# antoyang/TubeDETR

Measured on AMD Instinct MI355X. Metric: training clips/sec (fwd+bwd) at T=100 k=4 res=352, 1/2/4/8 MI355X, higher is better.
Workload: dtype bf16

## Files before the change

### include/tubedetr_hip.h

```cpp
#ifndef TUBEDETR_HIP_H
#define TUBEDETR_HIP_H
#include <stddef.h>
#include <stdint.h>
#ifdef __cplusplus
extern "C" {
#endif

#define TD_F32 0
#define TD_BF16 1
#define TD_U8 2
#define TD_OK 0
#define TD_ERR_INVALID (-1)
#define TD_ERR_LAUNCH (-2)

typedef void* td_stream_t;

const char* td_last_error(void);
int td_abi_version(void);

int td_set_deterministic(int on);
int td_get_deterministic(void);


#define TD_PROF_GEMM_128x128 0
#define TD_PROF_GEMM_128x64 1
#define TD_PROF_WGRAD 2
#define TD_PROF_GEMM_64x128 3
#define TD_PROF_PW_RESIDENT 4
#define TD_PROF_GEMM_256 5
#define TD_PROF_GEMM_256_PW 6
#define TD_PROF_FUSED 7
#define TD_PROF_CROSS_Q1 8
#define TD_PROF_WGRAD_SINGLE 9
#define TD_PROF_CHAIN 10
#define TD_PROF_FAMILIES 11
int td_prof_enable(int on);
int td_prof_collect(int family, int dtype, long long* launches, double* ms, double* flops);
int td_prof_collect_bytes(int family, int dtype, double* bytes);
int td_prof_dump(const char* path);
int td_debug_set_stamp_buffer(unsigned long long* buf);

typedef struct td_conv_desc {
  int N, Hs, Ws, C;
  int Ho, Wo;
  int R, S, stride, pad;
  int mode;
  int Nc;
  int ldc;
  int out_sp;
  int out_H, out_W;
  int aniso;
  int stride_w, pad_w;
} td_conv_desc;

typedef struct td_epilogue {
  const float* bias;
  const void* residual;
  const void* mask_src;
  int relu;
  int sigmoid;
  float dropout_p;
  uint32_t dropout_seed;
  float alpha;
  const uint32_t* dropout_counter;
} td_epilogue;

int td_conv_gemm(const void* src, const void* wmat, void* out, const td_conv_desc* d, const td_epilogue* e,
                 int dtype, td_stream_t stream);

typedef struct td_linear_ex_desc {
  int M, N, K1, K2;
  int lda1, lda2, ldc, ldr;
  int w_shared;
  long long rows1, rows2;
  const int* a1_map;
  const int* a2_map;
  const int* out_map;
  const int* res_map;
} td_linear_ex_desc;
int td_linear_ex(const void* a1, const void* a2, const void* wmat, void* out, const td_linear_ex_desc* x, const td_epilogue* e,
                 int dtype, td_stream_t stream);

int td_conv_wgrad(const void* g, const void* src, float* dw, const td_conv_desc* d, int ldg, int dtype, int splits,
                  td_stream_t stream);
int td_conv_wgrad_bias(const void* g, const void* src, float* dw, float* dbias, const td_conv_desc* d, int ldg, int dtype,
                       int splits, td_stream_t stream);

typedef struct td_wgrad_job {
  const void* g;
  const void* src;
  float* dW;
  const float* scale;
  td_conv_desc d;
  int ldg;
  int ci_real;
  float* dbias;
  int accumulate;
  int prezeroed;
} td_wgrad_job;
size_t td_conv_wgrad_batch_table_bytes(int n_jobs);
int td_conv_wgrad_batch(const td_wgrad_job* jobs, int n_jobs, int dtype, void* table_host, void* table_dev, size_t table_bytes,
                        td_stream_t stream);

typedef struct td_frame_source {
  const void* data;
  int dtype;
  int n;
  const int* index;
  const int* valid_hw;
} td_frame_source;
int td_frames_to_nhwc(const td_frame_source* srcs, int n_srcs, int C, int H, int W, int Cpad, const float* mean,
                      const float* inv_std, void* y, int dtype, td_stream_t stream);

size_t td_resnet_fwd_ws_bytes(int N, int H, int W, const int* nblocks, int dtype, int save);
int td_resnet_num_convs(const int* nblocks);
int td_resnet_fwd(const td_frame_source* srcs, int n_srcs, const float* mean, const float* inv_std, int N, int H, int W,
                  const int* nblocks, const void* const* w_fwd, const float* const* bias, int save, void* ws, size_t ws_bytes,
                  void** feat, int* feat_hw, int stem_pairs, int first_train_stage, int dtype, td_stream_t stream);
int td_bottleneck_fused(const void* x, void* out, const void* w1, const float* b1, const void* w2, const float* b2, const void* w3,
                        const float* b3, const void* wd, const float* bd, int N, int H, int W, int Cin, int dtype, td_stream_t stream);
int td_pw_chain2(const void* y2, const void* w3, const float* b3, const void* residual, void* out, const void* w1, const float* b1,
                 void* h1, int M, int planes, int dtype, td_stream_t stream);
int td_stem_pair_weights(const void* w_fwd_8, void* w_pairs, int Co, int dtype, td_stream_t stream);
int td_stem_pool(const void* x_pairs, const void* w_pairs, const float* bias, void* pooled, int N, int H, int W, int dtype,
                 td_stream_t stream);
size_t td_resnet_bwd_ws_bytes(int N, int H, int W, const int* nblocks, int first_train_stage, int dtype);
size_t td_resnet_bwd_table_bytes(const int* nblocks, int first_train_stage);
int td_resnet_bwd(const void* dfeat, int N, int N_fwd, int H, int W, const int* nblocks, int first_train_stage,
                  const void* const* w_dgrad, const float* const* scale, float* const* dW, const void* fwd_ws, void* ws,
                  size_t ws_bytes, void* table_host, void* table_dev, size_t table_bytes, int dW_prezeroed, int dtype, int only_stage, td_stream_t stream);

int td_weight_prep(const float* W, const float* bn_w, const float* bn_b, const float* bn_rm, const float* bn_rv,
                   const float* bias, int Co, int Ci, int R, int S, int Cpad, void* w_fwd, void* w_dgrad,
                   float* bias_out, float* scale_out, int dtype, td_stream_t stream);

typedef struct td_prep_item {
  const float* W;
  const float *bn_w, *bn_b, *bn_rm, *bn_rv, *bias;
  void *w_fwd, *w_dgrad;
  float *bias_out, *scale_out;
  int Co, Ci, RS, Cpad, Co_alloc, blk0;
} td_prep_item;
int td_weight_prep_batch(const td_prep_item* items_dev, int n, int total_blocks, int dtype, td_stream_t stream);

int td_wgrad_finalize(const float* dw_k, const float* scale, float* dW, int Co, int Ci, int R, int S, int Cpad,
                      int accumulate, td_stream_t stream);

int td_nchw_to_nhwc(const float* x, void* y, int N, int C, int H, int W, int Cpad, int dtype, td_stream_t stream);
int td_nhwc_to_nchw(const void* x, float* y, int N, int C, int H, int W, int dtype, td_stream_t stream);
int td_cast(const void* x, void* y, size_t n, int src_dtype, int dst_dtype, td_stream_t stream);

// ... 106 lines not shown
```

### tubedetr_amd/_hip.py

```python
from __future__ import annotations

import ctypes as C
import os

import torch

TD_F32, TD_BF16 = 0, 1
EXPECTED_ABI = 11
_LIB_PATH = os.environ.get("TD_HIP_LIB") or os.path.join(os.path.dirname(os.path.abspath(__file__)), "lib", "libtubedetr_hip.so")
_lib = None


class ConvDesc(C.Structure):
    _fields_ = [(n, C.c_int) for n in ("N", "Hs", "Ws", "C", "Ho", "Wo", "R", "S", "stride", "pad", "mode", "Nc", "ldc", "out_sp", "out_H", "out_W",
                                       "aniso", "stride_w", "pad_w")]


class PrepItem(C.Structure):
    _fields_ = [(n, C.c_void_p) for n in ("W", "bn_w", "bn_b", "bn_rm", "bn_rv", "bias", "w_fwd", "w_dgrad", "bias_out", "scale_out")] + \
               [(n, C.c_int) for n in ("Co", "Ci", "RS", "Cpad", "Co_alloc", "blk0")]


class WgradJob(C.Structure):
    _fields_ = [("g", C.c_void_p), ("src", C.c_void_p), ("dW", C.c_void_p), ("scale", C.c_void_p), ("d", ConvDesc), ("ldg", C.c_int), ("ci_real", C.c_int), ("dbias", C.c_void_p), ("accumulate", C.c_int), ("prezeroed", C.c_int)]


TD_U8 = 2


class FrameSource(C.Structure):
    _fields_ = [("data", C.c_void_p), ("dtype", C.c_int), ("n", C.c_int), ("index", C.c_void_p), ("valid_hw", C.c_void_p)]


class LinearExDesc(C.Structure):
    _fields_ = [(n, C.c_int) for n in ("M", "N", "K1", "K2", "lda1", "lda2", "ldc", "ldr", "w_shared")] + \
               [("rows1", C.c_longlong), ("rows2", C.c_longlong)] + [(n, C.c_void_p) for n in ("a1_map", "a2_map", "out_map", "res_map")]


class OptimSegment(C.Structure):
    _fields_ = [("begin", C.c_longlong), ("end", C.c_longlong), ("group", C.c_int), ("active", C.c_int)]


class ResampleJob(C.Structure):
    _fields_ = [("src", C.c_void_p), ("src_frame_stride", C.c_longlong)] + [(n, C.c_int) for n in ("src_pitch", "T", "sh", "sw", "flip", "rh", "rw", "wy", "wx", "wh", "ww")] + \
               [("dst", C.c_void_p)] + [(n, C.c_int) for n in ("planar", "frame_off", "H", "W")] + [("mask", C.c_void_p)]


class Epilogue(C.Structure):
    _fields_ = [
        ("bias", C.c_void_p),
        ("residual", C.c_void_p),
        ("mask_src", C.c_void_p),
        ("relu", C.c_int),
        ("sigmoid", C.c_int),
        ("dropout_p", C.c_float),
        ("dropout_seed", C.c_uint32),
        ("alpha", C.c_float),
        ("dropout_counter", C.c_void_p),
    ]


_P, _I, _F, _U32, _SZ = C.c_void_p, C.c_int, C.c_float, C.c_uint32, C.c_size_t
_SIGS = {
    "td_prof_enable": [_I],
    "td_prof_dump": [C.c_char_p],
    "td_debug_set_stamp_buffer": [_P],
    "td_prof_collect": [_I, _I, C.POINTER(C.c_longlong), C.POINTER(C.c_double), C.POINTER(C.c_double)],
    "td_prof_collect_bytes": [_I, _I, C.POINTER(C.c_double)],
    "td_conv_gemm": [_P, _P, _P, C.POINTER(ConvDesc), C.POINTER(Epilogue), _I, _P],
    "td_conv_wgrad": [_P, _P, _P, C.POINTER(ConvDesc), _I, _I, _I, _P],
    "td_conv_wgrad_bias": [_P, _P, _P, _P, C.POINTER(ConvDesc), _I, _I, _I, _P],
    "td_conv_wgrad_batch": [C.POINTER(WgradJob), _I, _I, _P, _P, _SZ, _P],
    "td_resnet_num_convs": [C.POINTER(C.c_int)],
    "td_resnet_fwd": [C.POINTER(FrameSource), _I, C.POINTER(C.c_float), C.POINTER(C.c_float), _I, _I, _I, C.POINTER(C.c_int), C.POINTER(_P), C.POINTER(_P), _I, _P, _SZ,
                      C.POINTER(_P), C.POINTER(C.c_int), _I, _I, _I, _P],
    "td_bottleneck_fused": [_P, _P, _P, _P, _P, _P, _P, _P, _P, _P, _I, _I, _I, _I, _I, _P],
    "td_stem_pair_weights": [_P, _P, _I, _I, _P],
    "td_stem_pool": [_P, _P, _P, _P, _I, _I, _I, _I, _P],
    "td_pw_chain2": [_P, _P, _P, _P, _P, _P, _P, _P, _I, _I, _I, _P],
    "td_set_deterministic": [_I],
    "td_get_deterministic": [],
    "td_frames_to_nhwc": [C.POINTER(FrameSource), _I, _I, _I, _I, _I, C.POINTER(C.c_float), C.POINTER(C.c_float), _P, _I, _P],
    "td_resnet_bwd": [_P, _I, _I, _I, _I, C.POINTER(C.c_int), _I, C.POINTER(_P), C.POINTER(_P), C.POINTER(_P), _P, _P, _SZ, _P, _P, _SZ, _I, _I, _I, _P],
    "td_weight_prep_batch": [_P, _I, _I, _I, _P],
    "td_weight_prep": [_P, _P, _P, _P, _P, _P, _I, _I, _I, _I, _I, _P, _P, _P, _P, _I, _P],
    "td_wgrad_finalize": [_P, _P, _P, _I, _I, _I, _I, _I, _I, _P],
    "td_nchw_to_nhwc": [_P, _P, _I, _I, _I, _I, _I, _I, _P],
    "td_nhwc_to_nchw": [_P, _P, _I, _I, _I, _I, _I, _P],
    "td_cast": [_P, _P, _SZ, _I, _I, _P],
    "td_maxpool3x3s2": [_P, _P, _I, _I, _I, _I, _I, _P],
    "td_add_layernorm_fwd": [_P, _P, _P, _P, _P, _P, _P, _P, _I, _I, _F, _I, _P],
    "td_add_layernorm_bwd": [_P, _P, _P, _P, _P, _P, _P, _P, _P, _I, _I, _I, _P],
    "td_colsum": [_P, _P, _I, _I, _I, _I, _P],
    "td_add": [_P, _P, _P, _SZ, _I, _P],
    "td_relu_bwd": [_P, _P, _P, _SZ, _F, _I, _P],
    "td_gelu_fwd": [_P, _P, _SZ, _I, _P],
    "td_gelu_bwd": [_P, _P, _P, _SZ, _I, _P],
    "td_dropout": [_P, _P, _SZ, _F, _U32, _P, _I, _P],
    "td_pos_sine": [_P, _P, _I, _I, _I, _I, _F, _I, _I, _P],
    "td_linear_ex": [_P, _P, _P, _P, C.POINTER(LinearExDesc), C.POINTER(Epilogue), _I, _P],
    "td_rows_copy": [_P, _P, _P, _P, _P, _I, _I, _I, _I, _I, _I, _P],
    "td_rows_segment_sum": [_P, _P, _P, _P, _P, _I, _I, _I, _I, _I, _P],
    "td_criterion_fwd": [_P, _P, _P, _P, _P, _P, _P, _P, _P, _F, _F, _I, _I, _I, _I, _P, _P, _P, _P, _P, _P],
    "td_criterion_bwd": [_P, _P, _P, _P, _P, _P, _P, _P, _I, _I, _I, _P],
    "td_sted_decode": [_P, _P, _I, _I, _P],
    "td_grad_norm_clip": [_P, _SZ, C.POINTER(OptimSegment), _I, _F, _P, _SZ, _P, _P, _P],
    "td_adamw_ema_step": [_P, _P, _P, _P, _P, _SZ, C.POINTER(OptimSegment), _I, _P, _P, _P, _F, _F, _F, _F, _F, _P],
    "td_mha_fwd": [_P, _P, _P, _P, _P, _P, _P, _I, _I, _I, _I, _I, _I, _I, _I, _I, _F, _F, _U32, _P, _I, _P],
    "td_mha_bwd": [_P, _P, _P, _P, _P, _P, _P, _P, _P, _P, _I, _I, _I, _I, _I, _I, _I, _I, _I, _F, _F, _U32, _P, _I, _P],
    "td_cross_q1_fwd": [_P, _P, _P, _P, _P, _P, _P, _I, _I, _I, _I, _I, _F, _U32, _P, _I, _P],
    "td_cross_q1_bwd": [_P, _P, _P, _P, _P, _P, _P, _P, _I, _I, _I, _I, _I, _I, _F, _U32, _P, _I, _P],
    "td_cross_q1_bwd_coef": [_P, _P, _P, _P, _P, _P, _P, _P, _I, _I, _I, _I, _I, _I, _I, _F, _U32, _P, _I, _P],
    "td_cross_q1_dmem": [_P, _I, _P, _P, _I, _P, _I, _I, _I, _I, _I, _I, _P],
    "td_head_blocks_expand": [_P, _P, _F, _P, _P, _I, _I, _I, _P],
    "td_head_blocks_extract": [_P, _F, _P, _P, _I, _I, _P],
    "td_mha_lean_fwd": [_P, _P, _P, _P, _P, _P, _I, _I, _I, _I, _I, _I, _I, _I, _I, _F, _F, _U32, _P, _I, _P],
    "td_mha_lean_bwd": [_P, _P, _P, _P, _P, _P, _P, _P, _P, _P, _I, _I, _I, _I, _I, _I, _I, _I, _I, _F, _F, _U32, _P, _I, _P],
    "td_clip_resample": [C.POINTER(ResampleJob), _I, _P, _P, _SZ, _P],
}
_SIZE_SIGS = {
    "td_grad_norm_ws_bytes": [],
    "td_mha_lean_stats_bytes": [_I, _I, _I],
    "td_conv_wgrad_batch_table_bytes": [_I],
    "td_clip_resample_table_bytes": [_I],
    "td_resnet_bwd_table_bytes": [C.POINTER(C.c_int), _I],
    "td_resnet_fwd_ws_bytes": [_I, _I, _I, C.POINTER(C.c_int), _I, _I],
    "td_resnet_bwd_ws_bytes": [_I, _I, _I, C.POINTER(C.c_int), _I, _I],
}
EXPORTS = ["td_last_error", "td_abi_version"] + list(_SIGS) + list(_SIZE_SIGS)


def lib_path() -> str:
    return _LIB_PATH


def lib() -> C.CDLL:
    global _lib
    if _lib is None:
        if not os.path.exists(_LIB_PATH):
            raise RuntimeError(
                f"{_LIB_PATH} is missing: build it with `python -m tubedetr_amd.build` (or __graft_entry__.build()); "
                "tubedetr_amd has no CPU / eager fallback"
            )
        L = C.CDLL(_LIB_PATH)
        L.td_last_error.restype = C.c_char_p
        L.td_last_error.argtypes = []
        L.td_abi_version.restype = C.c_int
        L.td_abi_version.argtypes = []
        got = L.td_abi_version()
        if got != EXPECTED_ABI:
            raise RuntimeError(f"{_LIB_PATH} has ABI version {got}, this binding needs {EXPECTED_ABI}: rebuild it with "
                               "`python -m tubedetr_amd.build --force`")
# ... 35 lines not shown
```

### tubedetr_amd/csrc/gemm_conv.hip

```cpp
#include <stdlib.h>

#include <type_traits>

#include "td_common.h"
#include <algorithm>
#include <vector>

#ifndef TD_WGRAD_EARLY_ISSUE
#define TD_WGRAD_EARLY_ISSUE 1
#endif
#ifndef TD_BIG_XCD_CONTIG
#define TD_BIG_XCD_CONTIG 1
#endif
namespace td {

struct GemmParams {
  const char* src;
  const char* w;
  char* out;
  td_conv_desc d;
  int M, K;
  uint32_t src_bytes, w_bytes;
  unsigned long long* dbg;
  const float* bias;
  const char* residual;
  const char* mask_src;
  int relu, sigmoid;
  float alpha;
  uint32_t drop_thresh;
  float drop_scale;
  uint32_t seed;
  const uint32_t* seed_dev;
  const char* src2;
  uint32_t src2_bytes;
  int K1, lda1, lda2, ldr;
  int w_shared;
  const int* a1_map;
  const int* a2_map;
  const int* out_map;
  const int* res_map;
  int tap_inner;
  int w_ld;
  int wtap[4];
  int use_wtap;
};

template <typename T>
struct Mfma;
template <>
struct Mfma<u16> {
  static __device__ __forceinline__ void run(const uint4& wf, const uint4& af, f32x4& acc) {
    acc = __builtin_amdgcn_mfma_f32_16x16x32_bf16(*(const bf16x8*)&wf, *(const bf16x8*)&af, acc, 0, 0, 0);
  }
};
template <>
struct Mfma<float> {
  static __device__ __forceinline__ void run(const uint4& wf, const uint4& af, f32x4& acc) {
    const float* a = (const float*)&wf;
    const float* b = (const float*)&af;
#pragma unroll
    for (int s = 0; s < 4; ++s) acc = __builtin_amdgcn_mfma_f32_16x16x4f32(a[s], b[s], acc, 0, 0, 0);
  }
};

template <typename T>
__device__ __forceinline__ void load4(const char* base, size_t off, float (&o)[4]);
template <>
__device__ __forceinline__ void load4<float>(const char* base, size_t off, float (&o)[4]) {
  float4 v = *(const float4*)(base + off * 4);
  o[0] = v.x; o[1] = v.y; o[2] = v.z; o[3] = v.w;
}
template <>
__device__ __forceinline__ void load4<u16>(const char* base, size_t off, float (&o)[4]) {
  uint2 v = *(const uint2*)(base + off * 2);
  o[0] = __uint_as_float(v.x << 16); o[1] = __uint_as_float(v.x & 0xffff0000u);
  o[2] = __uint_as_float(v.y << 16); o[3] = __uint_as_float(v.y & 0xffff0000u);
}
template <typename T, typename V>
__device__ __forceinline__ void unpack4(const V& v, float (&o)[4]);
template <>
__device__ __forceinline__ void unpack4<float, float4>(const float4& v, float (&o)[4]) {
  o[0] = v.x; o[1] = v.y; o[2] = v.z; o[3] = v.w;
}
template <>
__device__ __forceinline__ void unpack4<u16, uint2>(const uint2& v, float (&o)[4]) {
  o[0] = __uint_as_float(v.x << 16); o[1] = __uint_as_float(v.x & 0xffff0000u);
  o[2] = __uint_as_float(v.y << 16); o[3] = __uint_as_float(v.y & 0xffff0000u);
}
typedef __bf16 bf16x2_t __attribute__((ext_vector_type(2)));
__device__ __forceinline__ uint32_t pack_bf16x2(float lo, float hi) {
  bf16x2_t v = {(__bf16)lo, (__bf16)hi};
  return *(uint32_t*)&v;
}
template <typename T>
__device__ __forceinline__ void unpack16(const uint4& v, float (&o)[16 / sizeof(T)]);
template <>
__device__ __forceinline__ void unpack16<float>(const uint4& v, float (&o)[4]) {
  o[0] = __uint_as_float(v.x); o[1] = __uint_as_float(v.y); o[2] = __uint_as_float(v.z); o[3] = __uint_as_float(v.w);
}
template <>
__device__ __forceinline__ void unpack16<u16>(const uint4& v, float (&o)[8]) {
  o[0] = __uint_as_float(v.x << 16); o[1] = __uint_as_float(v.x & 0xffff0000u);
  o[2] = __uint_as_float(v.y << 16); o[3] = __uint_as_float(v.y & 0xffff0000u);
  o[4] = __uint_as_float(v.z << 16); o[5] = __uint_as_float(v.z & 0xffff0000u);
  o[6] = __uint_as_float(v.w << 16); o[7] = __uint_as_float(v.w & 0xffff0000u);
}
template <typename T>
__device__ __forceinline__ uint4 pack16(const float (&v)[16 / sizeof(T)]);
template <>
__device__ __forceinline__ uint4 pack16<float>(const float (&v)[4]) {
  return make_uint4(__float_as_uint(v[0]), __float_as_uint(v[1]), __float_as_uint(v[2]), __float_as_uint(v[3]));
}
template <>
__device__ __forceinline__ uint4 pack16<u16>(const float (&v)[8]) {
  return make_uint4(pack_bf16x2(v[0], v[1]), pack_bf16x2(v[2], v[3]), pack_bf16x2(v[4], v[5]), pack_bf16x2(v[6], v[7]));
}
template <typename T>
__device__ __forceinline__ void store4(char* base, size_t off, const float (&v)[4]);
template <>
__device__ __forceinline__ void store4<float>(char* base, size_t off, const float (&v)[4]) {
  *(float4*)(base + off * 4) = make_float4(v[0], v[1], v[2], v[3]);
}
template <>
__device__ __forceinline__ void store4<u16>(char* base, size_t off, const float (&v)[4]) {
  uint2 o;
  o.x = (uint32_t)f32_to_bf16(v[0]) | ((uint32_t)f32_to_bf16(v[1]) << 16);
  o.y = (uint32_t)f32_to_bf16(v[2]) | ((uint32_t)f32_to_bf16(v[3]) << 16);
  *(uint2*)(base + off * 2) = o;
}

__device__ __forceinline__ float sigmoidf_(float x) { return 1.f / (1.f + __expf(-x)); }

typedef __attribute__((address_space(3))) void* lds_ptr_t;

#ifndef TD_NT
#define TD_NT 3
#endif
typedef uint32_t u32x4_t __attribute__((ext_vector_type(4)));
typedef uint32_t u32x2_t __attribute__((ext_vector_type(2)));
__device__ __forceinline__ uint4 ld16(const char* p) {
#if TD_NT & 1
  const u32x4_t v = __builtin_nontemporal_load((const u32x4_t*)p);
  return make_uint4(v.x, v.y, v.z, v.w);
#else
  return *(const uint4*)p;
#endif
}
__device__ __forceinline__ void st16(char* p, const uint4& v) {
#if TD_NT & 2
  __builtin_nontemporal_store(u32x4_t{v.x, v.y, v.z, v.w}, (u32x4_t*)p);
#else
  *(uint4*)p = v;
#endif
}

template <typename T, int BM, int BN, int NST, bool PW, bool TU = false, bool GX = false>
__global__ __launch_bounds__(256, (BM * BN >= 128 * 128 || NST == 3) ? 2 : 3) void conv_gemm_kernel(GemmParams p) {
  static_assert(!(PW && TU), "pointwise layers have no taps");
  static_assert(!GX || (PW && NST == 2), "the gather-extended operand is a pointwise, two-stage instance");
  constexpr int ES = sizeof(T);
  constexpr int VEC = 16 / ES;
  constexpr int BK = 128 / ES;
  constexpr int AI = BM / 32, BI = BN / 32;
  constexpr int WM = BM / 2, WN = BN / 2;
  constexpr int TM = WM / 16, TN = WN / 16;
  constexpr uint32_t OOB = 0xFFFFFFF0u;
  __shared__ __attribute__((aligned(16))) char smem0[(BM + BN) * 128];
  __shared__ __attribute__((aligned(16))) char smem1[(BM + BN) * 128];
  __shared__ __attribute__((aligned(16))) char smem2[NST == 3 ? (BM + BN) * 128 : 16];

  const td_conv_desc& d = p.d;
  const int t = threadIdx.x;
  const int wave = __builtin_amdgcn_readfirstlane(t >> 6), lane = t & 63;
  const int NT = (d.Nc + BN - 1) / BN;
  const int xcd = blockIdx.x & 7, seq = blockIdx.x >> 3;
  const int mt = (seq / NT) * 8 + xcd, nt = seq - (seq / NT) * NT;
  const int m0 = mt * BM, n0 = nt * BN;
  if (m0 >= p.M) return;
  const int lrow = lane >> 3;
  const int chunk = (lane & 7) ^ lrow;
  const int HoWo = d.Ho * d.Wo;

  const __amdgpu_buffer_rsrc_t rs_src = __builtin_amdgcn_make_buffer_rsrc((void*)p.src, 0, p.src_bytes, 0x00020000);
  const __amdgpu_buffer_rsrc_t rs_w = __builtin_amdgcn_make_buffer_rsrc((void*)p.w, 0, p.w_bytes, 0x00020000);
  const __amdgpu_buffer_rsrc_t rs_src2 = __builtin_amdgcn_make_buffer_rsrc((void*)(GX ? p.src2 : p.src), 0, GX ? p.src2_bytes : p.src_bytes, 0x00020000);

  int a_img[AI], a_hb[AI], a_wb[AI];
  bool a_ok[AI];
  uint32_t a_off[AI];
  uint32_t a_off2[GX ? AI : 1];
  int a_base[AI];
  uint32_t a_mask[AI];
  const int RS = d.R * d.S;
#pragma unroll
  for (int i = 0; i < AI; ++i) {
    int m = m0 + (i * 4 + wave) * 8 + lrow;
    a_ok[i] = m < p.M;
    if constexpr (GX) {
      const int mm = a_ok[i] ? m : 0;
      const int r1 = p.a1_map ? p.a1_map[mm] : mm;
      const int r2 = p.a2_map ? p.a2_map[mm] : mm;
      a_off[i] = a_ok[i] ? (uint32_t)r1 * (uint32_t)p.lda1 * ES : OOB;
      a_off2[i] = (a_ok[i] && p.src2) ? (uint32_t)r2 * (uint32_t)p.lda2 * ES : OOB;
    } else if constexpr (PW) {
      a_off[i] = a_ok[i] ? (uint32_t)m * (uint32_t)p.K * ES : OOB;
    } else {
      int mm = a_ok[i] ? m : 0;
      int n = mm / HoWo;
      int rem = mm - n * HoWo;
      int ho = rem / d.Wo, wo = rem - ho * d.Wo;
      a_img[i] = n * d.Hs * d.Ws;
      if (d.mode == 0) {
        a_hb[i] = ho * d.stride - d.pad;
        a_wb[i] = d.aniso ? wo * d.stride_w - d.pad_w : wo * d.stride - d.pad;
      } else {
        a_hb[i] = ho + d.pad;
        a_wb[i] = wo + d.pad;
      }
      if constexpr (TU) {
        a_base[i] = a_img[i] + a_hb[i] * d.Ws + a_wb[i];
        uint32_t msk = 0;
        for (int r = 0; r < d.R; ++r) {
          const int hs = d.mode == 0 ? a_hb[i] + r : a_hb[i] - r;
          for (int sx = 0; sx < d.S; ++sx) {
            const int ws = d.mode == 0 ? a_wb[i] + sx : a_wb[i] - sx;
            const bool in = (unsigned)hs < (unsigned)d.Hs && (unsigned)ws < (unsigned)d.Ws;
            msk |= (in ? 1u : 0u) << (r * d.S + sx);
          }
        }
        a_mask[i] = a_ok[i] ? msk : 0u;
      }
    }
  }
  uint32_t b_off[BI];
#pragma unroll
  for (int i = 0; i < BI; ++i) {
    int n = n0 + (i * 4 + wave) * 8 + lrow;
    b_off[i] = n < d.Nc ? (uint32_t)n * (uint32_t)(p.w_ld ? p.w_ld : ((GX && p.w_shared) ? p.K1 : p.K)) * ES : OOB;
  }
// ... 163 lines not shown
    for (int kt = 0; kt < nk; kt += 2) {
      __syncthreads();
      if (kt == 0) TD_STAMP(1);
      if (kt + 1 < nk) issue_tile(smem1);
      compute_tile(smem0);
      if (kt + 1 >= nk) break;
      __syncthreads();
      if (kt + 2 < nk) issue_tile(smem0);
      compute_tile(smem1);
    }
    TD_STAMP(2);
    fetch_epilogue_operands();
  } else {
#define TD_CG_STEP(cur, nxt, j)                                                     \
  asm volatile("s_waitcnt vmcnt(%0)" ::"n"(AI + BI) : "memory");                    \
  __builtin_amdgcn_s_barrier();                                                     \
  issue_tile(nxt);                                                                  \
  if ((j) >= 0) compute_tile(cur);
    for (int it = -2; it < nk; it += 3) {
      TD_CG_STEP(smem1, smem0, it)
      if (it + 1 >= nk) break;
      TD_CG_STEP(smem2, smem1, it + 1)
      if (it + 2 >= nk) break;
      TD_CG_STEP(smem0, smem2, it + 2)
    }
#undef TD_CG_STEP
    asm volatile("s_waitcnt vmcnt(0)" ::: "memory");
    TD_STAMP(2);
    fetch_epilogue_operands();
  }

  asm volatile("s_waitcnt lgkmcnt(0)" ::: "memory");
  __builtin_amdgcn_s_barrier();
  TD_STAMP(3);
  float* stg = (float*)((wave < 2 ? smem0 : smem1) + (wave & 1) * (WM * WN * 4));
  const float alpha = p.alpha;
#pragma unroll
  for (int j = 0; j < TM; ++j) {
    const int row = j * 16 + lr;
#pragma unroll
    for (int i = 0; i < TN; ++i) {
      const int c = (i * 4 + lg) ^ (row & (CPRW - 1));
      f32x4 a = acc[i][j];
      *(float4*)(stg + row * WN + c * 4) = make_float4(a[0] * alpha, a[1] * alpha, a[2] * alpha, a[3] * alpha);
    }
  }
  asm volatile("s_waitcnt lgkmcnt(0)" ::: "memory");
  float bias[EPL];
#pragma unroll
  for (int r = 0; r < EPL; ++r) bias[r] = (p.bias && n + r < d.Nc) ? p.bias[n + r] : 0.f;
  TD_STAMP(4);
  const uint32_t eff_seed = effective_seed(p.seed, p.drop_thresh ? p.seed_dev : nullptr);
#pragma unroll
  for (int it = 0; it < NIT; ++it) {
    if (!live[it]) continue;
    const int row = it * RPI + rsub;
    const int sw = row & (CPRW - 1);
    float v[EPL];
#pragma unroll
    for (int q = 0; q < EPL / 4; ++q) {
      float4 f = *(const float4*)(stg + row * WN + (((cc * (EPL / 4) + q) ^ sw) * 4));
      v[4 * q + 0] = f.x + bias[4 * q + 0]; v[4 * q + 1] = f.y + bias[4 * q + 1];
      v[4 * q + 2] = f.z + bias[4 * q + 2]; v[4 * q + 3] = f.w + bias[4 * q + 3];
    }
    const size_t off = offs[it];
    if (vec_ok) {
      if (p.residual) {
        float r8[EPL];
        unpack16<T>(res[it], r8);
#pragma unroll
        for (int r = 0; r < EPL; ++r) v[r] += r8[r];
      }
      if (p.relu) {
#pragma unroll
        for (int r = 0; r < EPL; ++r) v[r] = fmaxf(v[r], 0.f);
      }
      if (p.sigmoid) {
#pragma unroll
        for (int r = 0; r < EPL; ++r) v[r] = sigmoidf_(v[r]);
      }
      if (p.mask_src) {
        float m8[EPL];
        unpack16<T>(msk[it], m8);
#pragma unroll
        for (int r = 0; r < EPL; ++r) v[r] = m8[r] > 0.f ? v[r] : 0.f;
      }
      if (p.drop_thresh) {
#pragma unroll
        for (int r = 0; r < EPL; ++r) v[r] = dropout_keep(eff_seed, (uint32_t)(off + r), p.drop_thresh) ? v[r] * p.drop_scale : 0.f;
      }
      st16(p.out + off * ES, pack16<T>(v));
    } else {
      const int cnt = min(EPL, d.Nc - n);
      for (int r = 0; r < cnt; ++r) {
        float x = v[r];
        if (p.residual) x += Elem<T>::load(p.residual, (GX ? roffs[it] : off) + r);
        if (p.relu) x = fmaxf(x, 0.f);
        if (p.sigmoid) x = sigmoidf_(x);
        if (p.mask_src) x = Elem<T>::load(p.mask_src, off + r) > 0.f ? x : 0.f;
        if (p.drop_thresh) x = dropout_keep(eff_seed, (uint32_t)(off + r), p.drop_thresh) ? x * p.drop_scale : 0.f;
        Elem<T>::store(p.out, off + r, x);
      }
    }
  }
  TD_STAMP(5);
#undef TD_STAMP
}

#ifndef TD_ABL
#define TD_ABL 0
#endif
template <int OFF>
__device__ __forceinline__ u32x4_t lds_read16(uint32_t addr) {
  u32x4_t r;
#if TD_ABL & 4
  asm volatile("" : "=v"(r) : "v"(addr));
#else
  asm volatile("ds_read_b128 %0, %1 offset:%2" : "=v"(r) : "v"(addr), "n"(OFF));
#endif
  return r;
}
template <int N>
__device__ __forceinline__ void wait_vmcnt() {
  asm volatile("s_waitcnt vmcnt(%0)" ::"n"(N) : "memory");
}
template <int I>
using ic = std::integral_constant<int, I>;

#ifndef TD_BIG8_AUX_W
#define TD_BIG8_AUX_W 0
#endif
#ifndef TD_BIG8_AUX_X
#define TD_BIG8_AUX_X 0
#endif
template <bool TU, bool RES>
__global__ __launch_bounds__(512, 1) void conv_gemm_big8_kernel(GemmParams p) {
  using T = u16;
  constexpr int ES = 2, BM = 256, BN = 256, BK = 64, NW = 8, VEC = 8;
  constexpr int WM = 128, WN = 64, TM = 8, TN = 4;
  constexpr int STAGE = (BM + BN) * 128, WREG = BM * 128;
  constexpr uint32_t OOB = 0xFFFFFFF0u;
  constexpr int MAXT = 160;
  constexpr int STG = 16 * WN * ES;
  __shared__ __attribute__((aligned(16))) char smem[2 * STAGE];
  __shared__ __attribute__((aligned(16))) uint4 ktab[MAXT];
  __shared__ __attribute__((aligned(16))) char stg_all[NW * STG];

  const td_conv_desc& d = p.d;
  const int t = threadIdx.x;
  const int wave = __builtin_amdgcn_readfirstlane(t >> 6), lane = t & 63;
  const int NT = d.Nc / BN;
  const int lrow = lane >> 3;
  const int chunk = (lane & 7) ^ lrow;
  const int HoWo = d.Ho * d.Wo;
  const __amdgpu_buffer_rsrc_t rs_src = __builtin_amdgcn_make_buffer_rsrc((void*)p.src, 0, p.src_bytes, 0x00020000);
  const __amdgpu_buffer_rsrc_t rs_w = __builtin_amdgcn_make_buffer_rsrc((void*)p.w, 0, p.w_bytes, 0x00020000);
  const uint32_t out_bytes = (uint32_t)p.M * (uint32_t)d.ldc * ES;
  const __amdgpu_buffer_rsrc_t rs_out = __builtin_amdgcn_make_buffer_rsrc((void*)p.out, 0, out_bytes, 0x00020000);
  const int wy = wave >> 2, wx = wave & 3;
  const int RS = d.R * d.S;
  const int lane_c = chunk * VEC;
  const int nk = p.K / BK;
  const bool tap_inner = TU && p.tap_inner;
  if (t < nk + 4) {
    uint32_t xo, tap = 0, wo;
    if constexpr (TU) {
      const int cpt = d.C / BK;
      const int chunkc = tap_inner ? t / RS : t % cpt;
// ... 185 lines not shown
#pragma unroll
    for (int i = 0; i < TN; ++i) bs[i] = p.bias ? *(const f32x4*)(p.bias + n0 + wx * WN + i * 16 + lg * 4) : f32x4{0.f, 0.f, 0.f, 0.f};
    wait_vmcnt<7>();
    __builtin_amdgcn_s_barrier();
    if (wy == 1) __builtin_amdgcn_s_barrier();
    TD_STAMP(1);
    const int npair = (nk + 1) / 2;
#pragma unroll 1
    for (int it = 0; it < npair; ++it) {
      phase(ic<0>{}, ic<0>{}); phase(ic<0>{}, ic<1>{}); phase(ic<0>{}, ic<2>{}); phase(ic<0>{}, ic<3>{});
      phase(ic<1>{}, ic<0>{}); phase(ic<1>{}, ic<1>{}); phase(ic<1>{}, ic<2>{}); phase(ic<1>{}, ic<3>{});
    }
    if (wy == 0) __builtin_amdgcn_s_barrier();
    TD_STAMP(2);
    asm volatile("s_waitcnt vmcnt(0) lgkmcnt(0)" ::: "memory");
    asm volatile("s_nop 15\n\ts_nop 15" ::: "memory");
#pragma unroll
    for (int i = 0; i < TN; ++i)
#pragma unroll
      for (int j = 0; j < TM; ++j) asm volatile("" : "+v"(acc[i][j]));
#pragma unroll
    for (int i = 0; i < TN; ++i) asm volatile("" : "+v"(bs[i]));
    const int vb_next = vb + (int)gridDim.x;
    const bool more = tile_ok(vb_next);
    if (more) {
      tile_addr(tile_m0(vb_next), tile_n0(vb_next));
      prologue_issue();
    }
    TD_STAMP(3);
    uint4 mk[2][2];
    auto seg_off = [&](int j, int h) -> uint32_t {
      const int m = m0 + wy * WM + j * 16 + h * 8 + rsub;
      return m < p.M ? ((uint32_t)m * (uint32_t)d.ldc + (uint32_t)(n0 + wx * WN + cc * 8)) * ES : OOB;
    };
    auto fetch_mask = [&](int j, int b) {
#pragma unroll
      for (int h = 0; h < 2; ++h) {
        const uint32_t off = seg_off(j, h);
        mk[b][h] = off != OOB ? ld16(p.mask_src + off) : make_uint4(0, 0, 0, 0);
      }
    };
    auto put = [&](int j) {
#pragma unroll
      for (int i = 0; i < TN; ++i) {
        const f32x4 a = acc[i][j];
        float v[4] = {a[0] * alpha + bs[i][0], a[1] * alpha + bs[i][1], a[2] * alpha + bs[i][2], a[3] * alpha + bs[i][3]};
        if constexpr (RES) {
          const int m = m0 + wy * WM + j * 16 + lr;
          if (m < p.M) {
            const uint2 rr = *(const uint2*)(p.residual + ((size_t)m * d.ldc + n0 + wx * WN + i * 16 + lg * 4) * ES);
            v[0] += __uint_as_float(rr.x << 16); v[1] += __uint_as_float(rr.x & 0xffff0000u);
            v[2] += __uint_as_float(rr.y << 16); v[3] += __uint_as_float(rr.y & 0xffff0000u);
          }
        }
        if (p.relu) {
#pragma unroll
          for (int r = 0; r < 4; ++r) v[r] = fmaxf(v[r], 0.f);
        }
        const uint32_t lo = pack_bf16x2(v[0], v[1]), hi = pack_bf16x2(v[2], v[3]);
        asm volatile("ds_write_b64 %0, %1" ::"v"(swa[i]), "v"(u32x2_t{lo, hi}) : "memory");
      }
    };
    if (p.mask_src) fetch_mask(0, 0);
    put(0);
    u32x4_t o0, o1;
    asm volatile("ds_read_b128 %0, %1" : "=v"(o0) : "v"(sra) : "memory");
    asm volatile("ds_read_b128 %0, %1 offset:1024" : "=v"(o1) : "v"(sra) : "memory");
#pragma unroll
    for (int j = 0; j < TM; ++j) {
      const int b = j & 1;
      if (j + 1 < TM) {
        if (p.mask_src) fetch_mask(j + 1, b ^ 1);
        put(j + 1);
        asm volatile("s_waitcnt lgkmcnt(4)" : "+v"(o0), "+v"(o1) : : "memory");
      } else {
        asm volatile("s_waitcnt lgkmcnt(0)" : "+v"(o0), "+v"(o1) : : "memory");
      }
      u32x4_t s0 = o0, s1 = o1;
      if (j + 1 < TM) {
        asm volatile("ds_read_b128 %0, %1" : "=v"(o0) : "v"(sra) : "memory");
        asm volatile("ds_read_b128 %0, %1 offset:1024" : "=v"(o1) : "v"(sra) : "memory");
      }
      if (p.mask_src) {
        float x8[8], m8[8];
        unpack16<T>(make_uint4(s0.x, s0.y, s0.z, s0.w), x8);
        unpack16<T>(mk[b][0], m8);
#pragma unroll
        for (int r = 0; r < 8; ++r) x8[r] = m8[r] > 0.f ? x8[r] : 0.f;
        const uint4 q0 = pack16<T>(x8);
        s0 = u32x4_t{q0.x, q0.y, q0.z, q0.w};
        unpack16<T>(make_uint4(s1.x, s1.y, s1.z, s1.w), x8);
        unpack16<T>(mk[b][1], m8);
#pragma unroll
        for (int r = 0; r < 8; ++r) x8[r] = m8[r] > 0.f ? x8[r] : 0.f;
        const uint4 q1 = pack16<T>(x8);
        s1 = u32x4_t{q1.x, q1.y, q1.z, q1.w};
      }
      __builtin_amdgcn_raw_buffer_store_b128(s0, rs_out, (int)seg_off(j, 0), 0, 0);
      __builtin_amdgcn_raw_buffer_store_b128(s1, rs_out, (int)seg_off(j, 1), 0, 0);
    }
    TD_STAMP(5);
    if (p.dbg && t == 0) p.dbg[(size_t)vb * 8 + 7] = wall_clock64();
    if (!more) break;
    vb = vb_next;
  }
#undef TD_STAMP
}

template <bool TU>
__global__ __launch_bounds__(512, 1) void conv_gemm_big8n_kernel(GemmParams p) {
  using T = u16;
  constexpr int ES = 2, BM = 256, BN = 128, BK = 64, NW = 8, VEC = 8;
  constexpr int WM = 64, WN = 64, TM = 4, TN = 4;
  constexpr int WREG = BM * 128, STAGE = (BM + BN) * 128;
  constexpr uint32_t OOB = 0xFFFFFFF0u;
  constexpr int MAXT = 160;
  __shared__ __attribute__((aligned(16))) char smem[3 * STAGE];
  __shared__ __attribute__((aligned(16))) uint4 ktab[MAXT];

  const td_conv_desc& d = p.d;
  const int t = threadIdx.x;
  const int wave = __builtin_amdgcn_readfirstlane(t >> 6), lane = t & 63;
  const int NT = d.Nc / BN;
  const int xcd = blockIdx.x & 7, seq = blockIdx.x >> 3;
#if TD_BIG_XCD_CONTIG
  const int mtx = (cdiv(p.M, BM) + 7) / 8;
  const int mt = xcd * mtx + seq / NT, nt = seq - (seq / NT) * NT;
#else
  const int mt = (seq / NT) * 8 + xcd, nt = seq - (seq / NT) * NT;
#endif
  const int m0 = mt * BM, n0 = nt * BN;
  if (m0 >= p.M) return;
  const int lrow = lane >> 3;
  const int chunk = (lane & 7) ^ lrow;
  const int lane_c = chunk * VEC;
  const int HoWo = d.Ho * d.Wo;
  const int RS = d.R * d.S;
  const __amdgpu_buffer_rsrc_t rs_src = __builtin_amdgcn_make_buffer_rsrc((void*)p.src, 0, p.src_bytes, 0x00020000);
  const __amdgpu_buffer_rsrc_t rs_w = __builtin_amdgcn_make_buffer_rsrc((void*)p.w, 0, p.w_bytes, 0x00020000);
  const int wy = wave >> 1, wx = wave & 1;
  const int grp = wave >> 2;

  uint32_t a_off[4], a_mask[4];
  const float rcp_howo = 1.f / (float)HoWo, rcp_wo = 1.f / (float)d.Wo;
  auto divmod = [](int a, int dv, float rcp, int& q, int& r) {
    q = (int)((float)a * rcp);
    r = a - q * dv;
    const int up = r >= dv, dn = r < 0;
    q += up - dn;
    r += (dn - up) * dv;
  };
#pragma unroll
  for (int q = 0; q < 4; ++q) {
    const int m = m0 + (wave >> 1) * WM + (q >> 1) * 32 + ((wave & 1) * 2 + (q & 1)) * 8 + lrow;
    const bool ok = m < p.M;
    if constexpr (!TU) {
      a_off[q] = ((uint32_t)m * (uint32_t)p.K + (uint32_t)lane_c) * ES;
      a_mask[q] = ok ? 1u : 0u;
    } else {
      const int mm = ok ? m : 0;
      int n, rem, ho, wo;
      divmod(mm, HoWo, rcp_howo, n, rem);
      divmod(rem, d.Wo, rcp_wo, ho, wo);
      const int hb = d.mode == 0 ? ho * d.stride - d.pad : ho + d.pad;
      const int wb = d.mode == 0 ? wo * d.stride - d.pad : wo + d.pad;
      a_off[q] = ((uint32_t)(n * d.Hs * d.Ws + hb * d.Ws + wb) * (uint32_t)d.C + (uint32_t)lane_c) * ES;
      uint32_t cols = 0, msk = 0;
      for (int sx = 0; sx < d.S; ++sx) cols |= ((unsigned)(d.mode == 0 ? wb + sx : wb - sx) < (unsigned)d.Ws ? 1u : 0u) << sx;
      for (int r = 0; r < d.R; ++r) msk |= ((unsigned)(d.mode == 0 ? hb + r : hb - r) < (unsigned)d.Hs ? cols : 0u) << (r * d.S);
      a_mask[q] = ok ? msk : 0u;
    }
  }
  uint32_t b_off[2];
#pragma unroll
  for (int i = 0; i < 2; ++i) b_off[i] = ((uint32_t)(n0 + (i * NW + wave) * 8 + lrow) * (uint32_t)p.K + (uint32_t)lane_c) * ES;
  const int nk = p.K / BK;
  const bool tap_inner = TU && p.tap_inner;
// ... 97 lines not shown
      if (p.residual) res[b][it] = ld16(p.residual + offs[b][it] * ES);
      if (p.mask_src) msk[b][it] = ld16(p.mask_src + offs[b][it] * ES);
    }
  };

#define TD_STAMP(i) do { if (p.dbg && t == 0) p.dbg[(size_t)blockIdx.x * 8 + (i)] = __builtin_readcyclecounter(); } while (0)
  TD_STAMP(0);
  __syncthreads();
  {
    const u32x4_t e0 = lds_read16<0>(tab0);
    const u32x4_t e1 = lds_read16<16>(tab0);
    e[2] = lds_read16<32>(tab0);
    asm volatile("s_waitcnt lgkmcnt(0)" ::: "memory");
    __builtin_amdgcn_sched_barrier(0);
    issue_w(smem, 0, e0); issue_w(smem, 1, e0); issue_x(smem, 0, e0); issue_x(smem, 1, e0); issue_x(smem, 2, e0); issue_x(smem, 3, e0);
    issue_w(smem + STAGE, 0, e1); issue_w(smem + STAGE, 1, e1); issue_x(smem + STAGE, 0, e1); issue_x(smem + STAGE, 1, e1);
    issue_x(smem + STAGE, 2, e1); issue_x(smem + STAGE, 3, e1);
  }
  wait_vmcnt<8>();
  __builtin_amdgcn_s_barrier();
  if (grp == 1) __builtin_amdgcn_s_barrier();
  TD_STAMP(1);
  const int ntri = (nk + 2) / 3;
#pragma unroll 1
  for (int it = 0; it < ntri; ++it) {
    phase(ic<0>{}, ic<0>{}); phase(ic<0>{}, ic<1>{});
    phase(ic<1>{}, ic<0>{}); phase(ic<1>{}, ic<1>{});
    phase(ic<2>{}, ic<0>{}); phase(ic<2>{}, ic<1>{});
  }
  if (grp == 0) __builtin_amdgcn_s_barrier();
  TD_STAMP(2);
  asm volatile("s_waitcnt vmcnt(0) lgkmcnt(0)" ::: "memory");
  asm volatile("s_nop 15\n\ts_nop 15" ::: "memory");
#pragma unroll
  for (int i = 0; i < TN; ++i)
#pragma unroll
    for (int j = 0; j < TM; ++j) asm volatile("" : "+v"(acc[i][j]));
  fetch_chunk(0, 0);
  __builtin_amdgcn_s_barrier();
  TD_STAMP(3);
  float* stg = (float*)(smem + wave * (CR * WN * 4));
  const float alpha = p.alpha;
  float bias[EPL];
#pragma unroll
  for (int r = 0; r < EPL; ++r) bias[r] = p.bias ? p.bias[n + r] : 0.f;
#pragma unroll
  for (int c = 0; c < NCH; ++c) {
    const int b = c & 1;
    {
      const int row = lr;
#pragma unroll
      for (int i = 0; i < TN; ++i) {
        const int cx = (i * 4 + lg) ^ (row & (CPRW - 1));
        const f32x4 a = acc[i][c];
        *(float4*)(stg + row * WN + cx * 4) = make_float4(a[0] * alpha, a[1] * alpha, a[2] * alpha, a[3] * alpha);
      }
    }
    if (c + 1 < NCH) fetch_chunk(c + 1, b ^ 1);
    asm volatile("s_waitcnt lgkmcnt(0)" ::: "memory");
#pragma unroll
    for (int it = 0; it < NIT; ++it) {
      const int row = it * RPI + rsub;
      const int sw = row & (CPRW - 1);
      float v[EPL];
#pragma unroll
      for (int q = 0; q < EPL / 4; ++q) {
        const float4 f = *(const float4*)(stg + row * WN + (((cc * (EPL / 4) + q) ^ sw) * 4));
        v[4 * q + 0] = f.x + bias[4 * q + 0]; v[4 * q + 1] = f.y + bias[4 * q + 1];
        v[4 * q + 2] = f.z + bias[4 * q + 2]; v[4 * q + 3] = f.w + bias[4 * q + 3];
      }
      if (p.residual) {
        float r8[EPL];
        unpack16<T>(res[b][it], r8);
#pragma unroll
        for (int r = 0; r < EPL; ++r) v[r] += r8[r];
      }
      if (p.relu) {
#pragma unroll
        for (int r = 0; r < EPL; ++r) v[r] = fmaxf(v[r], 0.f);
      }
      if (p.mask_src) {
        float m8[EPL];
        unpack16<T>(msk[b][it], m8);
#pragma unroll
        for (int r = 0; r < EPL; ++r) v[r] = m8[r] > 0.f ? v[r] : 0.f;
      }
      if (live[b][it]) st16(p.out + offs[b][it] * ES, pack16<T>(v));
    }
    asm volatile("s_waitcnt lgkmcnt(0)" ::: "memory");
  }
  TD_STAMP(5);
#undef TD_STAMP
}

template <int NKT, bool RES, bool MSK>
__global__ __launch_bounds__(256, 2) void pw_resident2_kernel(GemmParams p, int MT, int P) {
  using T = u16;
  constexpr int ES = 2;
  constexpr uint32_t OOB = 0xFFFFFFF0u;
  constexpr int WM = 32, WN = 64, TM = 2, TN = 4;
  constexpr int CPRW = WN / 4, EPL = 8, LPR = WN / EPL, RPI = 64 / LPR, NIT = WM / RPI;
  constexpr int NOPS = NIT * ((RES ? 1 : 0) + (MSK ? 1 : 0));
  constexpr bool AHEAD = NOPS > 0 && !(RES && MSK && NKT == 4);
  constexpr int NA = 2 * NKT;
  constexpr int AUX_NT = (TD_NT & 2) ? 2 : 0;
  __shared__ __attribute__((aligned(16))) char sA0[32768];
  __shared__ __attribute__((aligned(16))) char sA1[32768];
  __shared__ __attribute__((aligned(16))) char sT[4 * 16 * WN * 4];
  const td_conv_desc& d = p.d;
  const int t = threadIdx.x;
  const int wave = __builtin_amdgcn_readfirstlane(t >> 6), lane = t & 63;
  const int NT = d.Nc >> 7;
  const int xcd = blockIdx.x & 7, local = blockIdx.x >> 3;
  const int GPX = P / NT;
  const int nt = local % NT, gl = local / NT;
  if (gl >= GPX) return;
  const int gid = xcd * GPX + gl, G = 8 * GPX;
  const int lrow = lane >> 3, chunk = (lane & 7) ^ lrow;
  const uint32_t out_bytes = (uint32_t)p.M * (uint32_t)d.ldc * ES;
  const __amdgpu_buffer_rsrc_t rs_src = __builtin_amdgcn_make_buffer_rsrc((void*)p.src, 0, p.src_bytes, 0x00020000);
  const __amdgpu_buffer_rsrc_t rs_out = __builtin_amdgcn_make_buffer_rsrc((void*)p.out, 0, out_bytes, 0x00020000);
  const __amdgpu_buffer_rsrc_t rs_res = __builtin_amdgcn_make_buffer_rsrc((void*)(RES ? p.residual : p.out), 0, out_bytes, 0x00020000);
  const __amdgpu_buffer_rsrc_t rs_msk = __builtin_amdgcn_make_buffer_rsrc((void*)(MSK ? p.mask_src : p.out), 0, out_bytes, 0x00020000);
  const int n0 = nt * 128;
  const int HoWo = d.Ho * d.Wo;
  const bool strided = d.stride != 1;
  auto issue_A = [&](char* buf, int mt) {
    const int m0 = mt * 64;
    uint32_t row[2];
#pragma unroll
    for (int i = 0; i < 2; ++i) {
      const int m = m0 + (i * 4 + wave) * 8 + lrow;
      int src_row = m;
      if (strided) {
        const int img = m / HoWo, rem = m - img * HoWo;
        const int ho = rem / d.Wo, wo = rem - ho * d.Wo;
        src_row = (img * d.Hs + ho * d.stride) * d.Ws + wo * d.stride;
      }
      row[i] = (mt < MT && m < p.M) ? (uint32_t)src_row * (uint32_t)p.K * ES : OOB;
    }
#pragma unroll
    for (int kt = 0; kt < NKT; ++kt)
#pragma unroll
      for (int i = 0; i < 2; ++i) {
        const uint32_t off = row[i] != OOB ? row[i] + (uint32_t)(kt * 64 + chunk * 8) * ES : OOB;
        __builtin_amdgcn_raw_ptr_buffer_load_lds(rs_src, (lds_ptr_t)(buf + kt * 8192 + (i * 4 + wave) * 1024), 16, off, 0, 0, 0);
      }
  };
  const int wy = wave >> 1, wx = wave & 1;
  const int lr = lane & 15, lg = lane >> 4;
  const int cc = lane % LPR, rsub = lane / LPR;
  const int n = n0 + wx * WN + cc * EPL;
  float bias[EPL];
#pragma unroll
  for (int r = 0; r < EPL; ++r) bias[r] = p.bias ? p.bias[n + r] : 0.f;
  uint4 wfr[NKT][2][TN];
#pragma unroll
  for (int kt = 0; kt < NKT; ++kt)
#pragma unroll
    for (int ks = 0; ks < 2; ++ks)
#pragma unroll
      for (int i = 0; i < TN; ++i)
        wfr[kt][ks][i] = *(const uint4*)(p.w + ((size_t)(n0 + wx * WN + i * 16 + lr) * p.K + kt * 64 + ks * 32 + lg * 8) * ES);
  const uint32_t drop_seed = p.drop_thresh ? effective_seed(p.seed, p.seed_dev) : 0u;
  float* const stg = (float*)(sT + wave * (16 * WN * 4));

  auto seg_off = [&](int mt, int it) -> uint32_t {
    const int m = mt * 64 + wy * WM + it * RPI + rsub;
    return (mt < MT && m < p.M) ? ((uint32_t)m * (uint32_t)d.ldc + (uint32_t)n) * ES : OOB;
  };
  u32x4_t res[2][NIT], msk[2][NIT];
  auto fetch_ops = [&](int mt, int b) {
#pragma unroll
    for (int it = 0; it < NIT; ++it) {
      const uint32_t off = seg_off(mt, it);
      if constexpr (RES) asm volatile("buffer_load_dwordx4 %0, %1, %2, 0 offen nt" : "=v"(res[b][it]) : "v"(off), "s"(rs_res) : "memory");
      if constexpr (MSK) asm volatile("buffer_load_dwordx4 %0, %1, %2, 0 offen nt" : "=v"(msk[b][it]) : "v"(off), "s"(rs_msk) : "memory");
    }
  };

  auto step = [&](char* cur, char* nxt, int mt, auto B_) {
    constexpr int B = decltype(B_)::value;
    if constexpr (NOPS > 0 && !AHEAD) fetch_ops(mt, 0);
    wait_vmcnt<NA + NOPS>();
    __builtin_amdgcn_s_barrier();
    f32x4 acc[TN][TM];
#pragma unroll
    for (int i = 0; i < TN; ++i)
#pragma unroll
      for (int j = 0; j < TM; ++j) acc[i][j] = f32x4{0.f, 0.f, 0.f, 0.f};
#pragma unroll
    for (int kt = 0; kt < NKT; ++kt)
#pragma unroll
      for (int ks = 0; ks < 2; ++ks) {
        const int cidx = ks * 4 + lg;
        uint4 af[TM];
#pragma unroll
        for (int j = 0; j < TM; ++j) {
          const int row = wy * WM + j * 16 + lr;
          af[j] = *(const uint4*)(cur + kt * 8192 + row * 128 + ((cidx ^ (row & 7)) << 4));
        }
#pragma unroll
        for (int i = 0; i < TN; ++i)
#pragma unroll
          for (int j = 0; j < TM; ++j) Mfma<T>::run(wfr[kt][ks][i], af[j], acc[i][j]);
      }
    asm volatile("s_waitcnt lgkmcnt(0)" ::: "memory");
    __builtin_amdgcn_s_barrier();
    issue_A(cur, mt + 2 * G);
    if constexpr (AHEAD) fetch_ops(mt + G, B ^ 1);
    if constexpr (NOPS > 0) {
      wait_vmcnt<NA + (AHEAD ? NOPS : 0)>();
      __builtin_amdgcn_sched_barrier(0);
    }
    constexpr int RB = AHEAD ? B : 0;
#pragma unroll
    for (int j = 0; j < TM; ++j) {
#pragma unroll
      for (int i = 0; i < TN; ++i) {
        const int c = (i * 4 + lg) ^ (lr & (CPRW - 1));
        const f32x4 a = acc[i][j];
        *(float4*)(stg + lr * WN + c * 4) = make_float4(a[0], a[1], a[2], a[3]);
      }
      asm volatile("s_waitcnt lgkmcnt(0)" ::: "memory");
#pragma unroll
      for (int h = 0; h < 16 / RPI; ++h) {
        const int it = j * (16 / RPI) + h;
        const int row = h * RPI + rsub;
        const int sw = row & (CPRW - 1);
        float v[EPL];
#pragma unroll
        for (int q = 0; q < EPL / 4; ++q) {
          const float4 f = *(const float4*)(stg + row * WN + (((cc * (EPL / 4) + q) ^ sw) * 4));
          v[4 * q + 0] = f.x + bias[4 * q + 0]; v[4 * q + 1] = f.y + bias[4 * q + 1];
          v[4 * q + 2] = f.z + bias[4 * q + 2]; v[4 * q + 3] = f.w + bias[4 * q + 3];
        }
        const uint32_t off = seg_off(mt, it);
        if constexpr (RES) {
          float r8[EPL];
          unpack16<T>(make_uint4(res[RB][it].x, res[RB][it].y, res[RB][it].z, res[RB][it].w), r8);
#pragma unroll
          for (int r = 0; r < EPL; ++r) v[r] += r8[r];
        }
        if (p.relu) {
#pragma unroll
          for (int r = 0; r < EPL; ++r) v[r] = fmaxf(v[r], 0.f);
        }
        if constexpr (MSK) {
          float m8[EPL];
          unpack16<T>(make_uint4(msk[RB][it].x, msk[RB][it].y, msk[RB][it].z, msk[RB][it].w), m8);
#pragma unroll
          for (int r = 0; r < EPL; ++r) v[r] = m8[r] > 0.f ? v[r] : 0.f;
        }
        if (p.drop_thresh) {
#pragma unroll
          for (int r = 0; r < EPL; ++r) v[r] = dropout_keep(drop_seed, off / ES + (uint32_t)r, p.drop_thresh) ? v[r] * p.drop_scale : 0.f;
        }
        const uint4 o = pack16<T>(v);
        __builtin_amdgcn_raw_buffer_store_b128(u32x4_t{o.x, o.y, o.z, o.w}, rs_out, (int)off, 0, AUX_NT);
      }
      asm volatile("s_waitcnt lgkmcnt(0)" ::: "memory");
    }
  };

  int mt = gid;
  issue_A(sA0, mt);
  issue_A(sA1, mt + G);
  if constexpr (AHEAD) fetch_ops(mt, 0);
  while (mt < MT) {
    step(sA0, sA1, mt, ic<0>{});
    mt += G;
    if (mt >= MT) break;
    step(sA1, sA0, mt, ic<1>{});
    mt += G;
  }
  asm volatile("s_waitcnt vmcnt(0)" ::: "memory");
}

struct WgradParams {
  const char* g;
  const char* src;
  float* dw;
  const float* scale;
  float* dbias;
  td_conv_desc d;
  int M, K, ldg, mper;
  uint32_t g_bytes, src_bytes;
  int out_mode;
  int ci_real;
  int tn, tk, first;
  int cls;
  unsigned long long* stamps;
};

typedef __bf16 bf16x4 __attribute__((ext_vector_type(4)));

template <int ES>
__device__ __forceinline__ int wg_swz(int row) {
  return ES == 2 ? ((row & 3) | (((row >> 3) & 1) << 2)) : (row & 7);
}

template <typename T, int NSTG, bool PW>
__device__ __forceinline__ void wgrad_body(const WgradParams& p, const int bx, const int by, const int bz, const int lin) {
  constexpr int ES = sizeof(T);
  constexpr int VEC = 16 / ES;
  constexpr int MK = 128 / ES;
  constexpr int ROWB = 128 * ES;
  constexpr int CPR = ROWB / 16;
  constexpr int RPI = 64 / CPR;
  constexpr int LI = MK / (4 * RPI);
  constexpr int SWS = ES == 2 ? 1 : 2;
  constexpr int TILEB = MK * ROWB;
  constexpr uint32_t OOB = 0xFFFFFFF0u;
  __shared__ __attribute__((aligned(16))) char stage0[2 * TILEB];
  __shared__ __attribute__((aligned(16))) char stage1[2 * TILEB];
  __shared__ __attribute__((aligned(16))) char stage2[NSTG == 4 ? 2 * TILEB : 16];
  __shared__ __attribute__((aligned(16))) char stage3[NSTG == 4 ? 2 * TILEB : 16];

  const td_conv_desc& d = p.d;
  const int t = threadIdx.x;
  const int wave = __builtin_amdgcn_readfirstlane(t >> 6), lane = t & 63;
  const unsigned long long t_start = __builtin_readcyclecounter();
  const int co0 = bx * 128, kk0 = by * 128;
  const int mbeg = bz * p.mper;
  const int mend = min(p.M, mbeg + p.mper);
  if (mbeg >= mend) return;
  const int HoWo = d.Ho * d.Wo;
  constexpr bool pointwise = PW;
  const __amdgpu_buffer_rsrc_t rs_g = __builtin_amdgcn_make_buffer_rsrc((void*)p.g, 0, p.g_bytes, 0x00020000);
  const __amdgpu_buffer_rsrc_t rs_x = __builtin_amdgcn_make_buffer_rsrc((void*)p.src, 0, p.src_bytes, 0x00020000);

  int rloc[LI], gcol[LI], xr[LI], xs[LI], xc[LI];
  bool gok[LI], xok[LI];
#pragma unroll
  for (int i = 0; i < LI; ++i) {
// ... 648 lines not shown
  if (jok[Jx]) {                                                                                                                            \
    float v_[4];                                                                                                                            \
    asm volatile("v_accvgpr_read_b32 %0, a%c4\n\tv_accvgpr_read_b32 %1, a%c5\n\tv_accvgpr_read_b32 %2, a%c6\n\tv_accvgpr_read_b32 %3, a%c7"     \
                 : "=v"(v_[0]), "=v"(v_[1]), "=v"(v_[2]), "=v"(v_[3])                                                                        \
                 : "n"(4 * (8 * (I) + (Jx))), "n"(4 * (8 * (I) + (Jx)) + 1), "n"(4 * (8 * (I) + (Jx)) + 2), "n"(4 * (8 * (I) + (Jx)) + 3));      \
    float* dst = jdst[Jx] + (size_t)((I) * 16) * cstride;                                                                                   \
    _Pragma("unroll") for (int rr = 0; rr < 4; ++rr) {                                                                                      \
      const float v = v_[rr] * sc[I][rr];                                                                                                   \
      if (plain) dst[(size_t)rr * cstride] = v;                                                                                             \
      else atomicAdd(dst + (size_t)rr * cstride, v);                                                                                        \
    }                                                                                                                                       \
  }
  const size_t cstride = (size_t)p.ci_real * RS;
  bool jok[8];
  float* jdst[8];
#pragma unroll
  for (int j = 0; j < 8; ++j) {
    const int kko = kk0 + wxk * 128 + j * 16 + lr;
    int tap = 0, ci = kko;
    if (!PW && RS > 1) {
      tap = kko / d.C;
      ci = kko - tap * d.C;
    }
    jok[j] = kko < p.K && ci < p.ci_real;
    jdst[j] = p.dw + ((size_t)(co0 + wyc * 128 + 4 * lg) * p.ci_real + ci) * RS + tap;
  }
#define TD_W4_OUTROW(I) TD_W4_OUT(I, 0) TD_W4_OUT(I, 1) TD_W4_OUT(I, 2) TD_W4_OUT(I, 3) TD_W4_OUT(I, 4) TD_W4_OUT(I, 5) TD_W4_OUT(I, 6) TD_W4_OUT(I, 7)
  TD_W4_OUTROW(0) TD_W4_OUTROW(1) TD_W4_OUTROW(2) TD_W4_OUTROW(3) TD_W4_OUTROW(4) TD_W4_OUTROW(5) TD_W4_OUTROW(6) TD_W4_OUTROW(7)
#undef TD_W4_OUTROW
#undef TD_W4_OUT
}

__global__ __launch_bounds__(256, 1) void conv_wgrad_wide4_batch_kernel(const WgradParams* __restrict__ jobs, WgradXcdIndex xi) {
  __shared__ __attribute__((aligned(1024))) char w4s0[32768];
  __shared__ __attribute__((aligned(1024))) char w4s1[32768];
  __shared__ __attribute__((aligned(1024))) char w4s2[32768];
  __shared__ __attribute__((aligned(1024))) char w4s3[32768];
  const int xcd = blockIdx.x & 7, slot = blockIdx.x >> 3;
  if (slot >= xi.slots[xcd]) return;
  int lo = xi.start[xcd], hi = xi.start[xcd + 1] - 1;
  while (lo < hi) {
    const int mid = (lo + hi + 1) >> 1;
    if (jobs[mid].first <= slot) lo = mid;
    else hi = mid - 1;
  }
  const WgradParams p = jobs[lo];
  int local = slot - p.first;
  const int bx = local % p.tn;
  local /= p.tn;
  const int by = local % p.tk, bz = local / p.tk;
  if (p.cls & 4) wgrad_wide4_body<true>(p, bx, by, bz, w4s0, w4s1, w4s2, w4s3);
  else wgrad_wide4_body<false>(p, bx, by, bz, w4s0, w4s1, w4s2, w4s3);
}

static int validate(const td_conv_desc* d, int dtype, const char* who) {
  const int vec = dtype == TD_BF16 ? 8 : 4;
  TD_REQUIRE(dtype == TD_F32 || dtype == TD_BF16, "%s: bad dtype %d", who, dtype);
  TD_REQUIRE(d->C % vec == 0, "%s: source channels C=%d must be a multiple of %d (pad them)", who, d->C, vec);
  TD_REQUIRE(d->N > 0 && d->Hs > 0 && d->Ws > 0 && d->Ho > 0 && d->Wo > 0 && d->R > 0 && d->S > 0 && d->stride > 0,
             "%s: bad geometry", who);
  TD_REQUIRE((double)d->N * d->Hs * d->Ws * d->C < 2147483647.0, "%s: source tensor exceeds 2^31 elements", who);
  TD_REQUIRE(!d->aniso || (d->mode == 0 && d->stride_w >= 1 && d->pad_w >= 0 && d->out_sp <= 1), "%s: anisotropic stride / padding is a forward-only geometry", who);
  return TD_OK;
}

}

using namespace td;

static thread_local unsigned long long* g_dbg = nullptr;
static int persist_min_tiles() {
  static const int v = [] { const char* e = getenv("TD_PW_PERSIST_MIN"); return e ? atoi(e) : 4; }();
  return v;
}
extern "C" int td_debug_set_stamp_buffer(unsigned long long* buf) { g_dbg = buf; return TD_OK; }

struct WeightSubset {
  int w_ld;
  int ntap;
  int wtap[4];
  size_t w_bytes;
};
static int conv_gemm_launch(const void* src, const void* wmat, void* out, const td_conv_desc* d, const td_epilogue* e, int dtype,
                            td_stream_t stream, const WeightSubset* sub);

static int conv_dgrad_s2_by_parity(const void* g, const void* w_dgrad, void* dx, const td_conv_desc* d, const td_epilogue* e, int dtype,
                                   td_stream_t stream) {
  const int Hg = d->Hs, Wg = d->Ws, Co = d->C, H = d->Ho, W = d->Wo;
  const size_t es = 2, wbytes = (size_t)d->Nc * 9 * Co * es;
  for (int ph = 0; ph < 2; ++ph)
    for (int pw = 0; pw < 2; ++pw) {
      const int nr = ph ? 2 : 1, ns = pw ? 2 : 1;
      const int rmap[2] = {ph ? 2 : 1, 0}, smap[2] = {pw ? 2 : 1, 0};
      td_conv_desc c = {d->N, Hg, Wg, Co, Hg, Wg, nr, ns, 1, 0, 0, d->Nc, d->ldc, 2, H, W};
      WeightSubset sub;
      memset(&sub, 0, sizeof(sub));
      sub.w_ld = 9 * Co;
      sub.ntap = nr * ns;
      for (int r = 0; r < nr; ++r)
        for (int s_ = 0; s_ < ns; ++s_) sub.wtap[r * ns + s_] = rmap[r] * 3 + smap[s_];
      const size_t ooff = ((size_t)ph * W + pw) * d->ldc * es;
      td_epilogue ec;
      memset(&ec, 0, sizeof(ec));
      if (e) ec = *e;
      if (ec.residual) ec.residual = (const char*)ec.residual + ooff;
      if (ec.mask_src) ec.mask_src = (const char*)ec.mask_src + ooff;
      const char* wp = (const char*)w_dgrad;
      if (sub.ntap == 1) {
        wp += (size_t)sub.wtap[0] * Co * es;
        sub.wtap[0] = 0;
      }
      sub.w_bytes = wbytes - (size_t)(wp - (const char*)w_dgrad);
      const int rc = conv_gemm_launch(g, wp, (char*)dx + ooff, &c, &ec, dtype, stream, &sub);
      if (rc) return rc;
    }
  return TD_OK;
}

extern "C" int td_conv_gemm(const void* src, const void* wmat, void* out, const td_conv_desc* d, const td_epilogue* e,
                            int dtype, td_stream_t stream) {
  TD_REQUIRE(src && wmat && out && d, "td_conv_gemm: null pointer");
  static const int parity = [] { const char* e_ = getenv("TD_DGRAD_S2_PARITY"); return e_ ? atoi(e_) : 1; }();
  if (parity && dtype == TD_BF16 && d->mode == 1 && d->stride == 2 && d->R == 3 && d->S == 3 && d->pad == 1 && !d->aniso && d->out_sp <= 1 &&
      d->Ho == 2 * d->Hs && d->Wo == 2 * d->Ws && d->C % 64 == 0 && d->ldc >= d->Nc && !(e && (e->dropout_p > 0.f || e->sigmoid))) {
    int rc = validate(d, dtype, "td_conv_gemm");
    if (rc) return rc;
    return conv_dgrad_s2_by_parity(src, wmat, out, d, e, dtype, stream);
  }
  return conv_gemm_launch(src, wmat, out, d, e, dtype, stream, nullptr);
}

static int conv_gemm_launch(const void* src, const void* wmat, void* out, const td_conv_desc* d, const td_epilogue* e, int dtype,
                            td_stream_t stream, const WeightSubset* sub) {
  TD_REQUIRE(src && wmat && out && d, "td_conv_gemm: null pointer");
  int rc = validate(d, dtype, "td_conv_gemm");
  if (rc) return rc;
  GemmParams p;
  memset(&p, 0, sizeof(p));
  p.src = (const char*)src;
  p.w = (const char*)wmat;
  p.out = (char*)out;
  p.d = *d;
  if (p.d.out_sp < 1) p.d.out_sp = 1;
  p.M = d->N * d->Ho * d->Wo;
  p.K = d->R * d->S * d->C;
  {
    const double es = dtype == TD_BF16 ? 2.0 : 4.0;
    const double sb = (double)d->N * d->Hs * d->Ws * d->C * es, wb = (double)d->Nc * p.K * es;
    TD_REQUIRE(sb < 4294967000.0 && wb < 4294967000.0, "td_conv_gemm: operand exceeds the 4 GiB buffer-descriptor range");
    p.src_bytes = (uint32_t)sb;
    p.w_bytes = (uint32_t)wb;
  }
  if (sub) {
    p.w_ld = sub->w_ld;
    p.w_bytes = (uint32_t)sub->w_bytes;
    p.use_wtap = sub->ntap > 1;
    for (int i = 0; i < 4; ++i) p.wtap[i] = sub->wtap[i];
  }
  p.alpha = 1.f;
  p.dbg = g_dbg;
  if (e) {
    p.bias = e->bias;
    p.residual = (const char*)e->residual;
    p.mask_src = (const char*)e->mask_src;
    p.relu = e->relu;
    p.sigmoid = e->sigmoid;
    if (e->alpha != 0.f) p.alpha = e->alpha;
    if (e->dropout_p > 0.f) {
      TD_REQUIRE(e->dropout_p < 1.f, "td_conv_gemm: dropout_p must be < 1");
      p.drop_thresh = (uint32_t)((double)e->dropout_p * 4294967296.0);
      if (p.drop_thresh == 0) p.drop_thresh = 1;
      p.drop_scale = 1.f / (1.f - e->dropout_p);
      p.seed = e->dropout_seed;
      p.seed_dev = e->dropout_counter;
    }
  }
  TD_REQUIRE(d->ldc >= d->Nc, "td_conv_gemm: ldc < Nc");
  hipStream_t st = (hipStream_t)stream;
  static const int n_cu = [] {
    int dev = 0, cus = 256;
    if (hipGetDevice(&dev) == hipSuccess) (void)hipDeviceGetAttribute(&cus, hipDeviceAttributeMultiprocessorCount, dev);
    return cus;
  }();
  {
    static const int persist = [] { const char* e_ = getenv("TD_PW_PERSIST"); return e_ ? atoi(e_) : 1; }();
    static const int persist_dropout = [] { const char* e_ = getenv("TD_PW_PERSIST_DROPOUT"); return e_ ? atoi(e_) : 1; }();
    const bool pw0 = d->R == 1 && d->S == 1 && d->pad == 0 && p.d.out_sp == 1 && !d->aniso &&
                     ((d->stride == 1 && d->Hs == d->Ho && d->Ws == d->Wo) ||
                      (d->stride > 1 && d->mode == 0 && (d->Ho - 1) * d->stride < d->Hs && (d->Wo - 1) * d->stride < d->Ws));
    const int NTp = d->Nc / 128, Pp = 2 * n_cu / 8;
    const bool shape_ok = pw0 && !p.w_ld && dtype == TD_BF16 && p.K % 64 == 0 && p.K <= 256 && d->Nc % 128 == 0 &&
                          (NTp == 1 || NTp == 2 || NTp == 4 || NTp == 8 || NTp == 16) && Pp >= NTp && d->ldc % 8 == 0 && !p.sigmoid &&
                          p.alpha == 1.f && n_cu % 8 == 0 && (!p.drop_thresh || persist_dropout) && (double)p.M * d->ldc < 2147483000.0;
    const int MTp = cdiv(p.M, 64);
    const int groups = shape_ok ? 8 * (Pp / NTp) : 1;
    if (persist && shape_ok && MTp >= persist_min_tiles() * groups && !(persist == 2 && p.mask_src) && !(persist == 3 && d->mode != 0)) {
      const bool prof_ = prof_on();
      if (prof_) {
        prof_begin(TD_PROF_PW_RESIDENT, dtype, 2.0 * p.M * d->Nc * p.K, st, p.M, d->Nc, p.K, d->R, d->stride, d->mode);
        const double es_ = 2.0;
        double by = ((double)p.M * p.K + (double)d->Nc * p.K + (double)p.M * d->Nc) * es_;
        if (p.residual) by += (double)p.M * d->Nc * es_;
        if (p.mask_src) by += (double)p.M * d->Nc * es_;
        prof_set_bytes(by);
      }
      const int nkt = p.K / 64;
      const bool hr = p.residual != nullptr, hm = p.mask_src != nullptr;
      dim3 g2(2 * n_cu);
#define TD_PWR(NK)                                                                               \
  do {                                                                                           \
    if (hr && hm) pw_resident2_kernel<NK, true, true><<<g2, 256, 0, st>>>(p, MTp, Pp);          \
    else if (hr) pw_resident2_kernel<NK, true, false><<<g2, 256, 0, st>>>(p, MTp, Pp);          \
    else if (hm) pw_resident2_kernel<NK, false, true><<<g2, 256, 0, st>>>(p, MTp, Pp);          \
    else pw_resident2_kernel<NK, false, false><<<g2, 256, 0, st>>>(p, MTp, Pp);                 \
  } while (0)
      if (nkt == 1) TD_PWR(1);
      else if (nkt == 2) TD_PWR(2);
      else if (nkt == 3) TD_PWR(3);
      else TD_PWR(4);
#undef TD_PWR
      if (prof_) prof_end(st);
      return check_launch("td_conv_gemm(pw_resident)");
    }
  }
  const bool narrow = d->Nc <= 64;
  const int tiles128 = cdiv(p.M, 128) * cdiv(d->Nc, 128);
  const bool small_m = !narrow && (tiles128 < 512 || p.K <= 512);
  const int BMsel = small_m ? 64 : 128, BNsel = narrow ? 64 : 128;
  const int MT = cdiv(p.M, BMsel), NTl = cdiv(d->Nc, BNsel);
  dim3 grid(8 * cdiv(MT, 8) * NTl);
  const bool prof = prof_on();
  const bool pw = d->R == 1 && d->S == 1 && d->stride == 1 && d->pad == 0 && p.d.out_sp == 1 && d->Hs == d->Ho && d->Ws == d->Wo;
  static const int tu_on = [] { const char* e_ = getenv("TD_CONV_TAP_UNIFORM"); return e_ ? atoi(e_) : 1; }();
  const int bk = dtype == TD_BF16 ? 64 : 32;
  const bool tu = (tu_on || p.use_wtap) && !pw && !d->aniso && (d->R * d->S > 1 || (d->stride > 1 && d->mode == 0)) && d->R * d->S <= 32 && d->C % bk == 0 &&
                  (p.d.out_sp == 1 || d->mode == 0) && (d->mode == 0 || d->stride == 1);
  TD_REQUIRE(tu || !p.use_wtap, "td_conv_gemm: a weight-column subset needs the tap-uniform addressing (C %% %d == 0, at most 32 taps)", bk);
  {
    static const int big_on = [] { const char* e_ = getenv("TD_CONV_BIG"); return e_ ? atoi(e_) : 1; }();
    static const int big_min = [] { const char* e_ = getenv("TD_CONV_BIG_MIN_WG"); return e_ ? atoi(e_) : 160; }();
    const int bnb = d->Nc % 256 == 0 ? 256 : 128;
    const int wgs = cdiv(p.M, 256) * (d->Nc / bnb);
    if (big_on && dtype == TD_BF16 && (pw || tu) && p.d.out_sp == 1 && !p.use_wtap && !p.w_ld && d->Nc % 128 == 0 && p.K % 64 == 0 && p.K >= 512 && d->ldc % 8 == 0 && !p.sigmoid &&
        !p.drop_thresh && wgs >= big_min && (double)p.M * d->ldc < 2147483000.0 &&
        p.K <= 64 * 154 && p.M < (1 << 24)) {
      if (prof) {
        prof_begin(tu ? TD_PROF_GEMM_256 : TD_PROF_GEMM_256_PW, dtype, 2.0 * p.M * d->Nc * p.K, st, p.M, d->Nc, p.K, d->R, d->stride, d->mode);
        double by = ((double)d->N * d->Hs * d->Ws * d->C + (double)d->Nc * p.K + (double)p.M * d->Nc) * 2.0;
        if (p.residual) by += (double)p.M * d->Nc * 2.0;
        if (p.mask_src) by += (double)p.M * d->Nc * 2.0;
        prof_set_bytes(by);
      }
      static const int tap_inner = [] { const char* e_ = getenv("TD_CONV_TAP_INNER"); return e_ ? atoi(e_) : 1; }();
      p.tap_inner = tu && tap_inner && d->R * d->S > 1;
      dim3 gb(8 * cdiv(cdiv(p.M, 256), 8) * (d->Nc / bnb));
      static const int persist8 = [] { const char* e_ = getenv("TD_CONV_BIG_PERSIST"); return e_ ? atoi(e_) : 1; }();
      if (bnb == 256) {
        const dim3 gp(persist8 && n_cu % 8 == 0 ? std::min((unsigned)n_cu, gb.x) : gb.x);
        if (tu && p.residual) conv_gemm_big8_kernel<true, true><<<gp, 512, 0, st>>>(p);
        else if (tu) conv_gemm_big8_kernel<true, false><<<gp, 512, 0, st>>>(p);
        else if (p.residual) conv_gemm_big8_kernel<false, true><<<gp, 512, 0, st>>>(p);
        else conv_gemm_big8_kernel<false, false><<<gp, 512, 0, st>>>(p);
      } else {
        if (tu) conv_gemm_big8n_kernel<true><<<gb, 512, 0, st>>>(p);
        else conv_gemm_big8n_kernel<false><<<gb, 512, 0, st>>>(p);
      }
      if (prof) prof_end(st);
      return check_launch("td_conv_gemm(256-row tiles)");
    }
  }
  if (prof) prof_begin(narrow ? TD_PROF_GEMM_128x64 : (small_m ? TD_PROF_GEMM_64x128 : TD_PROF_GEMM_128x128), dtype, 2.0 * p.M * d->Nc * p.K, st, p.M, d->Nc, p.K, d->R, d->stride, d->mode);
  if (prof) {
    const double es = dtype == TD_BF16 ? 2.0 : 4.0;
    const double rows_out = d->out_sp > 1 ? (double)d->N * d->out_H * d->out_W : (double)p.M;
    double by = ((double)d->N * d->Hs * d->Ws * d->C + (double)d->Nc * p.K + (double)p.M * d->Nc) * es;
    if (e && e->residual) by += rows_out * d->Nc * es;
    if (e && e->mask_src) by += rows_out * d->Nc * es;
    prof_set_bytes(by);
  }
#define TD_LAUNCH(TT, BMv, BNv)                                                                   \
  do {                                                                                            \
    if (pw) conv_gemm_kernel<TT, BMv, BNv, 2, true><<<grid, 256, 0, st>>>(p);                    \
    else if (tu) conv_gemm_kernel<TT, BMv, BNv, 2, false, true><<<grid, 256, 0, st>>>(p);        \
    else conv_gemm_kernel<TT, BMv, BNv, 2, false><<<grid, 256, 0, st>>>(p);                      \
  } while (0)
  static const int deep = [] { const char* e_ = getenv("TD_CONV_DEEP"); return e_ ? atoi(e_) : 1; }();
  const bool deep_ok = deep && small_m && (int)grid.x <= 2 * 256 && p.K >= 1024;
  if (dtype == TD_BF16) {
    if (narrow) TD_LAUNCH(u16, 128, 64);
    else if (deep_ok && pw) conv_gemm_kernel<u16, 64, 128, 3, true><<<grid, 256, 0, st>>>(p);
    else if (deep_ok && tu) conv_gemm_kernel<u16, 64, 128, 3, false, true><<<grid, 256, 0, st>>>(p);
    else if (deep_ok) conv_gemm_kernel<u16, 64, 128, 3, false><<<grid, 256, 0, st>>>(p);
    else if (small_m) TD_LAUNCH(u16, 64, 128);
    else TD_LAUNCH(u16, 128, 128);
  } else {
    if (narrow) TD_LAUNCH(float, 128, 64);
    else if (small_m) TD_LAUNCH(float, 64, 128);
    else TD_LAUNCH(float, 128, 128);
  }
#undef TD_LAUNCH
  if (prof) prof_end(st);
  return check_launch("td_conv_gemm");
}

extern "C" int td_linear_ex(const void* a1, const void* a2, const void* wmat, void* out, const td_linear_ex_desc* x, const td_epilogue* e,
                            int dtype, td_stream_t stream) {
  TD_REQUIRE(a1 && wmat && out && x, "td_linear_ex: null pointer");
  TD_REQUIRE(dtype == TD_F32 || dtype == TD_BF16, "td_linear_ex: bad dtype %d", dtype);
  const int vec = dtype == TD_BF16 ? 8 : 4, bk = dtype == TD_BF16 ? 64 : 32;
  const int es = dtype == TD_BF16 ? 2 : 4;
  const int K2 = a2 ? x->K2 : 0;
  TD_REQUIRE(x->M >= 1 && x->N >= 1 && x->K1 >= vec && K2 >= 0, "td_linear_ex: bad sizes");
  TD_REQUIRE(x->K1 % vec == 0 && K2 % vec == 0 && x->lda1 % vec == 0 && (!a2 || x->lda2 % vec == 0), "td_linear_ex: K1 / K2 / lda must be multiples of %d", vec);
  TD_REQUIRE(!a2 || x->K1 % bk == 0, "td_linear_ex: with a second source K1=%d must be a multiple of the K tile (%d)", x->K1, bk);
  TD_REQUIRE(x->lda1 >= x->K1 && (!a2 || x->lda2 >= K2) && x->ldc >= x->N, "td_linear_ex: row stride smaller than the row");
  TD_REQUIRE(x->rows1 >= 1 && (!a2 || x->rows2 >= 1) && (x->a1_map || x->rows1 >= x->M) && (!a2 || x->a2_map || x->rows2 >= x->M),
             "td_linear_ex: source has fewer rows than M and no row map");
  GemmParams p;
  memset(&p, 0, sizeof(p));
  p.src = (const char*)a1;
  p.src2 = (const char*)a2;
  p.w = (const char*)wmat;
  p.out = (char*)out;
  p.M = x->M;
  p.K = x->K1 + K2;
  p.K1 = x->K1;
  p.lda1 = x->lda1;
  p.lda2 = a2 ? x->lda2 : 0;
  p.ldr = x->ldr > 0 ? x->ldr : x->ldc;
  p.w_shared = (a2 && x->w_shared) ? 1 : 0;
  TD_REQUIRE(!p.w_shared || K2 == x->K1, "td_linear_ex: a shared weight needs K2 == K1");
  p.a1_map = x->a1_map;
  p.a2_map = a2 ? x->a2_map : nullptr;
  p.out_map = x->out_map;
  p.res_map = x->res_map;
  td_conv_desc d;
  memset(&d, 0, sizeof(d));
  d.N = 1; d.Hs = x->M; d.Ws = 1; d.C = p.K; d.Ho = x->M; d.Wo = 1; d.R = d.S = 1; d.stride = 1; d.Nc = x->N; d.ldc = x->ldc; d.out_sp = 1;
  p.d = d;
  {
    const double b1 = (double)x->rows1 * x->lda1 * es, b2 = a2 ? (double)x->rows2 * x->lda2 * es : 16.0, wb = (double)x->N * (p.w_shared ? x->K1 : p.K) * es;
    TD_REQUIRE(b1 < 4294967000.0 && b2 < 4294967000.0 && wb < 4294967000.0, "td_linear_ex: operand exceeds the 4 GiB buffer-descriptor range");
    p.src_bytes = (uint32_t)b1;
    p.src2_bytes = (uint32_t)b2;
    p.w_bytes = (uint32_t)wb;
  }
  p.alpha = 1.f;
  if (e) {
    p.bias = e->bias;
    p.residual = (const char*)e->residual;
    p.mask_src = (const char*)e->mask_src;
    p.relu = e->relu;
    p.sigmoid = e->sigmoid;
    if (e->alpha != 0.f) p.alpha = e->alpha;
    if (e->dropout_p > 0.f) {
      TD_REQUIRE(e->dropout_p < 1.f, "td_linear_ex: dropout_p must be < 1");
      p.drop_thresh = (uint32_t)((double)e->dropout_p * 4294967296.0);
      if (p.drop_thresh == 0) p.drop_thresh = 1;
      p.drop_scale = 1.f / (1.f - e->dropout_p);
      p.seed = e->dropout_seed;
      p.seed_dev = e->dropout_counter;
    }
  }
  hipStream_t st = (hipStream_t)stream;
  const bool narrow = x->N <= 64;
  const int tiles128 = cdiv(p.M, 128) * cdiv(x->N, 128);
  const bool small_m = !narrow && (tiles128 < 512 || p.K <= 512);
  const int BMsel = small_m ? 64 : 128, BNsel = narrow ? 64 : 128;
  dim3 grid(8 * cdiv(cdiv(p.M, BMsel), 8) * cdiv(x->N, BNsel));
  const bool prof = prof_on();
  if (prof) {
    prof_begin(narrow ? TD_PROF_GEMM_128x64 : (small_m ? TD_PROF_GEMM_64x128 : TD_PROF_GEMM_128x128), dtype, 2.0 * p.M * x->N * p.K, st, p.M, x->N, p.K, 1, 1, 2);
    double by = ((double)p.M * p.K + (double)x->N * p.K + (double)p.M * x->N) * es;
    if (p.residual) by += (double)p.M * x->N * es;
    if (p.mask_src) by += (double)p.M * x->N * es;
    prof_set_bytes(by);
  }
// ... 266 lines not shown
```

### tubedetr_amd/functional.py

```python
from __future__ import annotations

import math
from typing import Optional

import torch
from torch.autograd import Function

from . import ops

Tensor = torch.Tensor

_EPOCH = [0]


def invalidate_prepared():
    _EPOCH[0] += 1


class _PrepEntry:
    __slots__ = ("base_ref", "offset", "shape", "bn", "dtype", "need_dgrad", "cpad", "co_alloc", "res", "ver", "dims")


class _PrepRegistry:

# ... 129 lines not shown


_USES: dict = {}


def _leaf(p):
    if p is None or p.is_leaf:
        return p
    return p._base if (p._base is not None and p._base.is_leaf) else None


def _note_use(recording: bool, *params) -> None:
    _drop_stale_deferred()
    if not recording:
        return
    for p in params:
        q = _leaf(p)
        if q is not None and q.requires_grad:
            _USES[id(q)] = _USES.get(id(q), 0) + 1


def _can_defer(*params) -> bool:
    if not _DEFER_ON[0]:
        return False
    for p in params:
        if p is None:
            continue
        q = _leaf(p)
        if q is None:
            return False
        if not q.requires_grad:
            continue
        if _USES.get(id(q), 0) != 1 or q.grad is not None or q._backward_hooks or getattr(q, "_post_accumulate_grad_hooks", None):
            return False
    return True


def _flush_deferred_wgrads():
    with _DEFER_LOCK:
        jobs = list(_DEFER_JOBS)
        _DEFER_JOBS.clear()
        _USES.clear()
        _ARMED[0] = False
    if jobs:
        ops.linear_wgrad_batch(jobs)


def _drop_stale_deferred():
    if _ARMED[0]:
        with _DEFER_LOCK:
            _DEFER_JOBS.clear()
            _USES.clear()
            _ARMED[0] = False


def _arm():
    with _DEFER_LOCK:
        if _ARMED[0]:
            return
        _ARMED[0] = True
    torch.autograd.Variable._execution_engine.queue_callback(_flush_deferred_wgrads)


def _wgrad(g: Tensor, x: Tensor, defer: bool, *, want_bias: bool, out: Optional[Tensor] = None, dbias: Optional[Tensor] = None,
           x2: Optional[Tensor] = None):
    M, K = x.shape
    N = g.shape[1]
    dev = g.device
    if not defer:
        db = dbias if dbias is not None else (ops.zeros_f32(N, dev) if want_bias else None)
        dW = ops.linear_wgrad(g, x, out=out, dbias=db)
        if x2 is not None:
            ops.linear_wgrad(g, x2, out=dW)
        return dW, db
    dW = out if out is not None else torch.empty((N, K), dtype=torch.float32, device=dev)
    db = dbias if dbias is not None else (torch.empty(N, dtype=torch.float32, device=dev) if want_bias else None)
    with _DEFER_LOCK:
        _DEFER_JOBS.append((g, x, dW.data_ptr(), db.data_ptr() if db is not None else None))
        if x2 is not None:
            _DEFER_JOBS.append((g, x2, dW.data_ptr(), None, True))
    return dW, db


class LinearFn(Function):

    @staticmethod
    def forward(ctx, x, W, b, relu: bool, dropout_p: float, seed: int):
        _note_use(ctx.needs_input_grad[1], W, b)
        N = W.shape[0]
        vec = ops.vec_of(x.dtype)
        Np = ops.pad_to(N, vec)
        wf, wd, _, _ = prepared(W, x.dtype, pad_out=Np if Np != N else 0)
        bias = b.detach() if b is not None else None
        if bias is not None and Np != N:
            bias = torch.cat([bias, bias.new_zeros(Np - N)])
        y = ops.linear_fwd(x, wf, bias, relu=relu, dropout_p=dropout_p, seed=seed)
        ctx.save_for_backward(x, y if (relu or dropout_p > 0) else None, wd)
        ctx.cfg = (relu, dropout_p, seed, N, Np, b is not None)
        ctx.params = (W, b)
        return y[:, :N].contiguous() if Np != N else y

    @staticmethod
    def backward(ctx, dy):
        _arm()
        x, y, wd = ctx.saved_tensors
        relu, p, seed, N, Np, has_b = ctx.cfg
        dy = dy.contiguous()
        if Np != N:
            g = dy.new_zeros((dy.shape[0], Np))
            g[:, :N] = dy
            dy = g
        if relu:
            g = ops.relu_bwd(dy, y, 1.0 / (1.0 - p) if p > 0 else 1.0)
        elif p > 0:
            g = ops.dropout(dy, p, seed)
        else:
            g = dy
        dx = ops.linear_fwd(g, wd) if ctx.needs_input_grad[0] else None
        want_w, want_b = ctx.needs_input_grad[1], has_b and ctx.needs_input_grad[2]
        dW = db = None
        if want_w:
            dW_full, db_full = _wgrad(g, x, _can_defer(*ctx.params), want_bias=want_b)
            dW = dW_full[:N]
            db = db_full[:N] if want_b else None
        elif want_b:
            db = ops.colsum(g)[:N]
        return dx, dW, db, None, None, None


def linear(x, W, b=None, relu=False, dropout_p=0.0, training=False):
    p = dropout_p if training else 0.0
    return LinearFn.apply(x, W, b, relu, p, _seed() if p > 0 else 0)


class FFNFn(Function):

    @staticmethod
    def forward(ctx, x, W1, b1, W2, b2, p: float, seed1: int, seed2: int):
        _note_use(ctx.needs_input_grad[1], W1, b1, W2, b2)
        w1f, w1d, _, _ = prepared(W1, x.dtype)
        w2f, w2d, _, _ = prepared(W2, x.dtype)
        h = ops.linear_fwd(x, w1f, b1.detach(), relu=True, dropout_p=p, seed=seed1)
        y = ops.linear_fwd(h, w2f, b2.detach(), dropout_p=p, seed=seed2)
        ctx.save_for_backward(x, h, w1d, w2d)
        ctx.cfg = (p, seed1, seed2)
        ctx.params = (W1, b1, W2, b2)
        return y

    @staticmethod
    def backward(ctx, dy):
        _arm()
        x, h, w1d, w2d = ctx.saved_tensors
        p, seed1, seed2 = ctx.cfg
        defer = _can_defer(*ctx.params)
        g2 = ops.dropout(dy.contiguous(), p, seed2) if p > 0 else dy.contiguous()
        dW2, db2 = _wgrad(g2, h, defer, want_bias=True)
        dh = ops.linear_fwd(g2, w2d, mask_src=h, alpha=1.0 / (1.0 - p) if p > 0 else 1.0)
        dW1, db1 = _wgrad(dh, x, defer, want_bias=True)
        dx = ops.linear_fwd(dh, w1d) if ctx.needs_input_grad[0] else None
        return dx, dW1, db1, dW2, db2, None, None, None


def ffn(x, W1, b1, W2, b2, dropout_p=0.0, training=False):
    p = dropout_p if training else 0.0
    return FFNFn.apply(x, W1, b1, W2, b2, p, _seed() if p > 0 else 0, _seed() if p > 0 else 0)


class AddLayerNormFn(Function):

    @staticmethod
    def forward(ctx, x, r, gamma, beta, eps: float):
        y, s, mean, rstd = ops.add_layernorm_fwd(x, r, gamma.detach(), beta.detach(), eps)
        ctx.save_for_backward(s, mean, rstd, gamma.detach())
        ctx.has_r = r is not None
        return y

    @staticmethod
    def backward(ctx, dy):
        s, mean, rstd, gamma = ctx.saved_tensors
        ds, dg, db = ops.add_layernorm_bwd(dy.contiguous(), s, mean, rstd, gamma)
        return ds, (ds if ctx.has_r else None), dg, db, None


def add_layernorm(x, r, gamma, beta, eps=1e-5):
    return AddLayerNormFn.apply(x, r, gamma, beta, eps)


class AddFn(Function):

    @staticmethod
    def forward(ctx, a, b):
        return ops.add(a, b)

    @staticmethod
    def backward(ctx, g):
        return g, g


class MHAFn(Function):

    @staticmethod
    def forward(ctx, q_in, q_pos, k_in, v_in, W_in, b_in, W_out, b_out, key_pad, B, Lq, Lk, H, need_w, p_attn, seed_attn, p_out, seed_out):
        _note_use(ctx.needs_input_grad[4], W_in, b_in, W_out, b_out)
        E = q_in.shape[1]
        dt = q_in.dtype
        same_qk = k_in is None
        bi = b_in.detach()

        def proj(x_, w_, b_):
            return ops.linear_ex(x_, w_, b_, a2=q_pos, w_shared=True) if q_pos is not None else ops.linear_fwd(x_, w_, b_)

        if same_qk:
            wqk_f, wqk_d, _, _ = prepared(W_in[: 2 * E], dt)
            qk = proj(q_in, wqk_f, bi[: 2 * E]).view(B, Lq, 2 * E)
            q, k = qk[..., :E], qk[..., E:]
            wd_list = (wqk_d,)
        else:
            wq_f, wq_d, _, _ = prepared(W_in[:E], dt)
            wk_f, wk_d, _, _ = prepared(W_in[E : 2 * E], dt)
            q = proj(q_in, wq_f, bi[:E]).view(B, Lq, E)
            k = ops.linear_fwd(k_in, wk_f, bi[E : 2 * E]).view(B, Lk, E)
            wd_list = (wq_d, wk_d)
        wv_f, wv_d, _, _ = prepared(W_in[2 * E :], dt)
        v = ops.linear_fwd(v_in, wv_f, bi[2 * E :]).view(B, Lk, E)
        scale = 1.0 / math.sqrt(E // H)
        lean = not need_w and ops.mha_lean_ok(q, k, v, H)
        if lean:
            ctxv, probs, kp = ops.mha_lean_fwd(q, k, v, key_pad, H, scale, dropout_p=p_attn, seed=seed_attn)
            wavg = None
        else:
            ctxv, probs, wavg = ops.mha_fwd(q, k, v, key_pad, H, scale, need_wavg=need_w, dropout_p=p_attn, seed=seed_attn)
            kp = None
        wo_f, wo_d, _, _ = prepared(W_out, dt)
        out = ops.linear_fwd(ctxv.view(B * Lq, E), wo_f, b_out.detach(), dropout_p=p_out, seed=seed_out)
        ctx.save_for_backward(q_in, q_pos, k_in, v_in, q, k, v, probs, ctxv, wv_d, wo_d, *wd_list)
        ctx.lean, ctx.kp = lean, kp
        ctx.cfg = (B, Lq, Lk, H, E, same_qk, scale, p_attn, seed_attn, p_out, seed_out)
        ctx.params = (W_in, b_in, W_out, b_out)
        return out, (wavg if need_w else None)

    @staticmethod
    def backward(ctx, dout, dwavg):
        _arm()
        q_in, q_pos, k_in, v_in, q, k, v, probs, ctxv, wv_d, wo_d, *wd_list = ctx.saved_tensors
        B, Lq, Lk, H, E, same_qk, scale, p_attn, seed_attn, p_out, seed_out = ctx.cfg
        dt = q_in.dtype
        dev = q_in.device
        defer = _can_defer(*ctx.params)
        g = ops.dropout(dout.contiguous(), p_out, seed_out) if p_out > 0 else dout.contiguous()
        if defer:
            dW_in = torch.empty((3 * E, E), dtype=torch.float32, device=dev)
            db_in = torch.empty(3 * E, dtype=torch.float32, device=dev)
        else:
            dW_in = ops.zeros_f32((3 * E, E), dev)
            db_in = ops.zeros_f32(3 * E, dev)
        dW_out, db_out = _wgrad(g, ctxv.view(B * Lq, E), defer, want_bias=True)
        dctx = ops.linear_fwd(g, wo_d).view(B, Lq, E)
        if same_qk:
            dqk = torch.empty((B, Lq, 2 * E), dtype=dt, device=dev)
            dq, dk = dqk[..., :E], dqk[..., E:]
        else:
            dq = torch.empty((B, Lq, E), dtype=dt, device=dev)
            dk = torch.empty((B, Lk, E), dtype=dt, device=dev)
        dv = torch.empty((B, Lk, E), dtype=dt, device=dev)
        dwa = dwavg.contiguous().float() if dwavg is not None else None
        if ctx.lean:
            ops.mha_lean_bwd(q, k, v, ctx.kp, ctxv, dctx, probs, H, scale, dq, dk, dv, dropout_p=p_attn, seed=seed_attn)
        else:
            ops.mha_bwd(q, k, v, dctx, probs, dwa, H, scale, dq, dk, dv, dropout_p=p_attn, seed=seed_attn)
        dv2 = dv.view(B * Lk, E)
        _wgrad(dv2, v_in, defer, want_bias=True, out=dW_in[2 * E :], dbias=db_in[2 * E :])
        d_v_in = ops.linear_fwd(dv2, wv_d) if ctx.needs_input_grad[3] else None
        d_q_in = d_k_in = None
        need_q = ctx.needs_input_grad[0] or (q_pos is not None and ctx.needs_input_grad[1])
        if same_qk:
            dqk2 = dqk.view(B * Lq, 2 * E)
            _wgrad(dqk2, q_in, defer, want_bias=True, out=dW_in[: 2 * E], dbias=db_in[: 2 * E], x2=q_pos)
            if need_q:
                d_q_in = ops.linear_fwd(dqk2, wd_list[0])
        else:
            dq2, dk2 = dq.view(B * Lq, E), dk.view(B * Lk, E)
            _wgrad(dq2, q_in, defer, want_bias=True, out=dW_in[:E], dbias=db_in[:E], x2=q_pos)
            _wgrad(dk2, k_in, defer, want_bias=True, out=dW_in[E : 2 * E], dbias=db_in[E : 2 * E])
            if need_q:
                d_q_in = ops.linear_fwd(dq2, wd_list[0])
            if ctx.needs_input_grad[2]:
                d_k_in = ops.linear_fwd(dk2, wd_list[1])
        return (d_q_in if ctx.needs_input_grad[0] else None, d_q_in if (q_pos is not None and ctx.needs_input_grad[1]) else None, d_k_in, d_v_in,
                dW_in, db_in, dW_out, db_out) + (None,) * 10


class _CrossKVShared:

    def __init__(self, mem, pos, n_layers, E):
        self.mem, self.pos, self.n_layers, self.E = mem, pos, n_layers, E
        self.dK = self.dV = None
        self.written = set()
        self.wk_d = self.wv_d = None

    def grads(self, like):
        if self.dK is None:
            self.dK = torch.empty((self.mem.shape[0], self.n_layers * self.E), dtype=like.dtype, device=like.device)
            self.dV = torch.empty_like(self.dK)
        return self.dK, self.dV


class CrossKVFn(Function):

    @staticmethod
    def forward(ctx, mem, pos, shared, *w_and_b):
        E, dt = shared.E, mem.dtype
        Ws, bs = w_and_b[0::2], w_and_b[1::2]
        kf, vf, kd, vd = [], [], [], []
        for W in Ws:
            f, d_, _, _ = prepared(W[E : 2 * E], dt)
            kf.append(f); kd.append(d_)
            f, d_, _, _ = prepared(W[2 * E :], dt)
            vf.append(f); vd.append(d_)
        bk = torch.cat([b.detach()[E : 2 * E] for b in bs])
        bv = torch.cat([b.detach()[2 * E :] for b in bs])
        wk = torch.cat(kf, dim=0)
        K_all = ops.linear_ex(mem, wk, bk, a2=pos, w_shared=True) if pos is not None else ops.linear_fwd(mem, wk, bk)
        V_all = ops.linear_fwd(mem, torch.cat(vf, dim=0), bv)
        shared.wk_d, shared.wv_d = torch.cat(kd, dim=1), torch.cat(vd, dim=1)
        ctx.shared = shared
        ctx.set_materialize_grads(False)
        return K_all, V_all

    @staticmethod
    def backward(ctx, gK, gV):
        sh = ctx.shared
        assert gK is None and gV is None, "the consumers of CrossKVFn hand their gradients over through the shared buffers"
        if sh.dK is None:
            return (None,) * (3 + 2 * sh.n_layers)
        for l in range(sh.n_layers):
            if l not in sh.written:
                sh.dK[:, l * sh.E : (l + 1) * sh.E].zero_()
                sh.dV[:, l * sh.E : (l + 1) * sh.E].zero_()
        d_mem = d_pos = None
        need_pos = sh.pos is not None and ctx.needs_input_grad[1]
        if ctx.needs_input_grad[0] or need_pos:
            d_k = ops.linear_fwd(sh.dK, sh.wk_d)
            if need_pos:
                d_pos = d_k
            if ctx.needs_input_grad[0]:
                d_mem = ops.linear_fwd(sh.dV, sh.wv_d, residual=d_k, out=None if need_pos else d_k)
        return (d_mem, d_pos, None) + (None,) * (2 * sh.n_layers)


class MHAPreKVFn(Function):

    @staticmethod
    def forward(ctx, q_in, q_pos, K_all, V_all, W_in, b_in, W_out, b_out, key_pad, shared, layer, B, Lq, Lk, H, need_w, p_attn, seed_attn, p_out, seed_out):
        _note_use(ctx.needs_input_grad[4], W_in, b_in, W_out, b_out)
        E = q_in.shape[1]
        dt = q_in.dtype
        nl = shared.n_layers
        wq_f, wq_d, _, _ = prepared(W_in[:E], dt)
        if q_pos is not None:
            q = ops.linear_ex(q_in, wq_f, b_in.detach()[:E], a2=q_pos, w_shared=True).view(B, Lq, E)
        else:
            q = ops.linear_fwd(q_in, wq_f, b_in.detach()[:E]).view(B, Lq, E)
        k = K_all.view(B, Lk, nl * E)[..., layer * E : (layer + 1) * E]
        v = V_all.view(B, Lk, nl * E)[..., layer * E : (layer + 1) * E]
        scale = 1.0 / math.sqrt(E // H)
        ctxv, probs, wavg = ops.mha_fwd(q, k, v, key_pad, H, scale, need_wavg=need_w, dropout_p=p_attn, seed=seed_attn)
        wo_f, wo_d, _, _ = prepared(W_out, dt)
        out = ops.linear_fwd(ctxv.view(B * Lq, E), wo_f, b_out.detach(), dropout_p=p_out, seed=seed_out)
        ctx.save_for_backward(q_in, q_pos, q, K_all, V_all, probs, ctxv, wq_d, wo_d)
        ctx.cfg = (B, Lq, Lk, H, E, scale, p_attn, seed_attn, p_out, seed_out, layer)
        ctx.params = (W_in, b_in, W_out, b_out)
        ctx.shared = shared
        return out, (wavg if need_w else None)

    @staticmethod
    def backward(ctx, dout, dwavg):
        _arm()
        q_in, q_pos, q, K_all, V_all, probs, ctxv, wq_d, wo_d = ctx.saved_tensors
        B, Lq, Lk, H, E, scale, p_attn, seed_attn, p_out, seed_out, layer = ctx.cfg
        sh = ctx.shared
        nl = sh.n_layers
        dt, dev = q_in.dtype, q_in.device
        defer = _can_defer(*ctx.params)
        g = ops.dropout(dout.contiguous(), p_out, seed_out) if p_out > 0 else dout.contiguous()
        if defer:
            dW_in = torch.empty((3 * E, E), dtype=torch.float32, device=dev)
            db_in = torch.empty(3 * E, dtype=torch.float32, device=dev)
        else:
            dW_in = ops.zeros_f32((3 * E, E), dev)
            db_in = ops.zeros_f32(3 * E, dev)
        dW_out, db_out = _wgrad(g, ctxv.view(B * Lq, E), defer, want_bias=True)
        dctx = ops.linear_fwd(g, wo_d).view(B, Lq, E)
        dq = torch.empty((B, Lq, E), dtype=dt, device=dev)
        dK_all, dV_all = sh.grads(K_all)
        cols = slice(layer * E, (layer + 1) * E)
        k = K_all.view(B, Lk, nl * E)[..., cols]
        v = V_all.view(B, Lk, nl * E)[..., cols]
        dk = dK_all.view(B, Lk, nl * E)[..., cols]
        dv = dV_all.view(B, Lk, nl * E)[..., cols]
        dwa = dwavg.contiguous().float() if dwavg is not None else None
        ops.mha_bwd(q, k, v, dctx, probs, dwa, H, scale, dq, dk, dv, dropout_p=p_attn, seed=seed_attn)
        sh.written.add(layer)
        dq2 = dq.view(B * Lq, E)
        _wgrad(dq2, q_in, defer, want_bias=True, out=dW_in[:E], dbias=db_in[:E], x2=q_pos)
        _wgrad(dK_all[:, cols], sh.mem, defer, want_bias=True, out=dW_in[E : 2 * E], dbias=db_in[E : 2 * E], x2=sh.pos)
        _wgrad(dV_all[:, cols], sh.mem, defer, want_bias=True, out=dW_in[2 * E :], dbias=db_in[2 * E :])
        need_pos = q_pos is not None and ctx.needs_input_grad[1]
        d_q_in = ops.linear_fwd(dq2, wq_d) if (ctx.needs_input_grad[0] or need_pos) else None
        return (d_q_in if ctx.needs_input_grad[0] else None, d_q_in if need_pos else None, None, None, dW_in, db_in, dW_out, db_out) + (None,) * 12


class _CrossQ1Shared:

    def __init__(self, mem, pos, want_dmem=True):
        self.mem, self.pos = mem, pos
        self.dmem = None
        self.want_dmem = want_dmem
        self.n_layers = 0
        self.coef = None
        self.deferred = {}


class CrossMemFn(Function):

    @staticmethod
    def forward(ctx, mem, shared):
        ctx.shared = shared
        ctx.set_materialize_grads(False)
        return mem.new_empty(0)

    @staticmethod
    def backward(ctx, g):
        sh = ctx.shared
        assert g is None, "the consumers of CrossMemFn hand their gradient over through the shared buffer"
        if sh.coef is not None:
            assert sh.dmem is None
            E = sh.mem.shape[1]
            F_, H = next(iter(sh.deferred.values()))[0].shape[0], next(iter(sh.deferred.values()))[0].shape[1] // E
            for l in range(sh.n_layers):
                if l not in sh.deferred:
                    sh.coef[:, 16 * l : 16 * l + 16].zero_()
            d = ops.cross_q1_dmem(sh.coef, [sh.deferred.get(l) for l in range(sh.n_layers)], F_, sh.mem.shape[0] // F_, H, E)
            sh.coef, sh.deferred = None, {}
            return d, None
        if sh.dmem is None:
            return None, None
        d = sh.dmem if sh.mem.dtype == torch.float32 else ops.cast(sh.dmem, sh.mem.dtype)
        sh.dmem = None
        return d, None


class CrossQ1Fn(Function):

    @staticmethod
    def forward(ctx, q_in, q_pos, token, W_in, b_in, W_out, b_out, key_pad, shared, F, S, H, need_w, p_attn, seed_attn, p_out, seed_out):
        _note_use(ctx.needs_input_grad[3], W_in, b_in, W_out, b_out)
        E = q_in.shape[1]
        dt = q_in.dtype
        scale = 1.0 / math.sqrt(E // H)
        wq_f, wq_d, _, _ = prepared(W_in[:E], dt)
        bq = b_in.detach()[:E]
        q = ops.linear_ex(q_in, wq_f, bq, a2=q_pos, w_shared=True) if q_pos is not None else ops.linear_fwd(q_in, wq_f, bq)
        Wd, bd = W_in.detach(), b_in.detach()
        wk_n, wk_t = ops.head_blocks_expand(Wd[E : 2 * E], None, scale, H, dt)
        wv_n, wv_t = ops.head_blocks_expand(Wd[2 * E :], bd[2 * E :], 1.0, H, dt)
        u = ops.linear_fwd(q, wk_t)
        probs, wavg, zext = ops.cross_q1_fwd(u, shared.mem, shared.pos, key_pad, F, S, H, need_wavg=need_w, dropout_p=p_attn, seed=seed_attn)
        ctxv = ops.linear_fwd(zext, wv_n)
        wo_f, wo_d, _, _ = prepared(W_out, dt)
        out = ops.linear_fwd(ctxv, wo_f, b_out.detach(), dropout_p=p_out, seed=seed_out)
        ctx.save_for_backward(q_in, q_pos, q, u, probs, zext, ctxv, wq_d, wo_d, wk_n, wv_t)
        ctx.cfg = (F, S, H, E, scale, p_attn, seed_attn, p_out, seed_out)
        ctx.params = (W_in, b_in, W_out, b_out)
        ctx.shared = shared
        ctx.layer = shared.n_layers
        shared.n_layers += 1
        return out, (wavg if need_w else None)

    @staticmethod
    def backward(ctx, dout, dwavg):
        _arm()
        q_in, q_pos, q, u, probs, zext, ctxv, wq_d, wo_d, wk_n, wv_t = ctx.saved_tensors
        F, S, H, E, scale, p_attn, seed_attn, p_out, seed_out = ctx.cfg
        sh = ctx.shared
        dt, dev = q_in.dtype, q_in.device
        defer = _can_defer(*ctx.params)
        g = ops.dropout(dout.contiguous(), p_out, seed_out) if p_out > 0 else dout.contiguous()
        dW_in = torch.empty((3 * E, E), dtype=torch.float32, device=dev)
        db_in = torch.empty(3 * E, dtype=torch.float32, device=dev)
        dW_out, db_out = _wgrad(g, ctxv, defer, want_bias=True)
        dctx = ops.linear_fwd(g, wo_d)
        d_zext = ops.linear_fwd(dctx, wv_t)
        Gv = ops.linear_wgrad(dctx, zext)
        ops.head_blocks_extract(Gv, 1.0, dW_in[2 * E :], db_in[2 * E :], H)
        dwa = dwavg.contiguous().float() if dwavg is not None else None
        if sh.want_dmem and dt == torch.bfloat16 and _CROSS_DMEM_DEFER and sh.n_layers <= 8 and sh.dmem is None:
            if sh.coef is None:
                width = (16 * sh.n_layers + 31) // 32 * 32
                sh.coef = torch.empty((F * S, width), dtype=dt, device=dev)
                if width > 16 * sh.n_layers:
                    sh.coef[:, 16 * sh.n_layers :].zero_()
            d_u = ops.cross_q1_bwd_coef(u, sh.mem, sh.pos, probs, d_zext, dwa, sh.coef, 16 * ctx.layer, F, S, H, dropout_p=p_attn, seed=seed_attn)
            sh.deferred[ctx.layer] = (u, d_zext)
        else:
            first = sh.dmem is None
            if not sh.want_dmem:
                dmem = None
            elif first:
                dmem = sh.dmem = torch.empty((F * S, E), dtype=torch.float32, device=dev)
            else:
                dmem = sh.dmem
            d_u = ops.cross_q1_bwd(u, sh.mem, sh.pos, probs, d_zext, dwa, dmem, sh.want_dmem and not first, F, S, H, dropout_p=p_attn, seed=seed_attn)
        dq = ops.linear_fwd(d_u, wk_n)
        Gk = ops.linear_wgrad(q, d_u)
        ops.head_blocks_extract(Gk, scale, dW_in[E : 2 * E], None, H)
        db_in[E : 2 * E].zero_()
        if defer:
            _wgrad(dq, q_in, True, want_bias=True, out=dW_in[:E], dbias=db_in[:E], x2=q_pos)
        else:
            dW_in[:E].zero_()
            db_in[:E].zero_()
            _wgrad(dq, q_in, False, want_bias=True, out=dW_in[:E], dbias=db_in[:E], x2=q_pos)
        need_pos = q_pos is not None and ctx.needs_input_grad[1]
        d_q_in = ops.linear_fwd(dq, wq_d) if (ctx.needs_input_grad[0] or need_pos) else None
        return (d_q_in if ctx.needs_input_grad[0] else None, d_q_in if need_pos else None, None, dW_in, db_in, dW_out, db_out) + (None,) * 10


_CROSS_DMEM_DEFER = _os.environ.get("TD_CROSS_DMEM_DEFER", "1") != "0"


def cross_q1_memory(mem, pos):
    shared = _CrossQ1Shared(mem.detach(), None if pos is None else pos.detach(), want_dmem=mem.requires_grad and torch.is_grad_enabled())
    return CrossMemFn.apply(mem, shared), shared


def multihead_attention_q1(q_in, anchor, W_in, b_in, W_out, b_out, key_pad, F, S, H, need_weights=True, attn_dropout=0.0, out_dropout=0.0,
                           training=False, q_pos=None):
    pa = attn_dropout if training else 0.0
    po = out_dropout if training else 0.0
    token, shared = anchor
    return CrossQ1Fn.apply(q_in, q_pos, token, W_in, b_in, W_out, b_out, key_pad, shared, F, S, H, need_weights,
                           pa, _seed() if pa > 0 else 0, po, _seed() if po > 0 else 0)


def cross_kv(mem, pos, attn_modules):
    E = attn_modules[0].embed_dim
    shared = _CrossKVShared(mem, pos, len(attn_modules), E)
    flat = []
    for m in attn_modules:
        flat += [m.in_proj_weight, m.in_proj_bias]
    K_all, V_all = CrossKVFn.apply(mem, pos, shared, *flat)
    return K_all, V_all, shared


def multihead_attention_prekv(q_in, kv, layer, W_in, b_in, W_out, b_out, key_pad, B, Lq, Lk, H, need_weights=False, attn_dropout=0.0,
                              out_dropout=0.0, training=False, q_pos=None):
    pa = attn_dropout if training else 0.0
    po = out_dropout if training else 0.0
    K_all, V_all, shared = kv
    return MHAPreKVFn.apply(q_in, q_pos, K_all, V_all, W_in, b_in, W_out, b_out, key_pad, shared, layer, B, Lq, Lk, H, need_weights,
                            pa, _seed() if pa > 0 else 0, po, _seed() if po > 0 else 0)


class ReplicaMaps:

    def __init__(self, owner, n: int, hw: int, L: int, device):
        owner = owner.cpu().long()
        F, S = owner.numel(), hw + L
        i32 = lambda t_: t_.to(torch.int32).contiguous().to(device)
        p, l_ = torch.arange(hw), torch.arange(L)
        f = torch.arange(F)
        self.F, self.n, self.hw, self.L, self.S = F, n, hw, L, S
        self.vis_src = i32((owner[:, None] * S + p[None, :]).reshape(-1))
        self.vis_dst = i32((f[:, None] * S + p[None, :]).reshape(-1))
        self.txt_src = i32((owner[:, None] * S + hw + l_[None, :]).reshape(-1))
        self.txt_dst = i32((f[:, None] * S + hw + l_[None, :]).reshape(-1))
        self.all_src = i32((owner[:, None] * S + torch.arange(S)[None, :]).reshape(-1))
        c = torch.arange(n)
        self.iota_vis = i32(torch.arange(n * hw))
        self.clip_vis = i32((c[:, None] * S + p[None, :]).reshape(-1))
        self.clip_txt = i32((c[:, None] * S + hw + l_[None, :]).reshape(-1))
        order = torch.argsort(owner, stable=True)
        counts = torch.bincount(owner, minlength=n)
        starts = torch.cumsum(counts, 0) - counts

        def csr(cols, row_off):
            m = cols.numel()
            per = counts[:, None].expand(n, m).reshape(-1)
            ptr = torch.zeros(n * m + 1, dtype=torch.long)
            ptr[1:] = torch.cumsum(per, 0)
            idx = torch.empty(int(ptr[-1]), dtype=torch.long)
            for ci in range(n):
                fr = order[starts[ci] : starts[ci] + counts[ci]]
                blk = (fr[None, :] * S + row_off + cols[:, None]).reshape(-1)
                idx[ptr[ci * m] : ptr[ci * m] + blk.numel()] = blk
            return i32(idx), i32(ptr)

        self.seg_vis = csr(p, 0)
        self.seg_txt = csr(l_, hw)
        self.seg_all = csr(torch.arange(S), 0)


class ReplicateRowsFn(Function):

    @staticmethod
    def forward(ctx, mem, maps):
        out = torch.empty((maps.F * maps.S, mem.shape[1]), dtype=mem.dtype, device=mem.device)
        ops.rows_copy(mem, maps.all_src, out, None, maps.F * maps.S)
        ctx.maps, ctx.rows = maps, mem.shape[0]
        return out

    @staticmethod
    def backward(ctx, g):
        maps = ctx.maps
        g = g.contiguous()
        d_mem = torch.empty((ctx.rows, g.shape[1]), dtype=g.dtype, device=g.device)
        ops.rows_segment_sum(g, maps.seg_all[0], maps.seg_all[1], d_mem)
        return d_mem, None


class SlowFastAggregateFn(Function):

    @staticmethod
    def forward(ctx, mem, fast_mem, W, b, maps):
        _note_use(ctx.needs_input_grad[2], W, b)
        dt = mem.dtype
        wf, wd, _, _ = prepared(W, dt)
        frames = torch.empty((maps.F * maps.S, mem.shape[1]), dtype=dt, device=mem.device)
        ops.linear_ex(mem, wf, b.detach(), a1_map=maps.vis_src, a2=fast_mem, w_shared=True, residual=mem, res_map=maps.vis_src, out=frames, out_map=maps.vis_dst)
        ops.rows_copy(mem, maps.txt_src, frames, maps.txt_dst, maps.F * maps.L)
        ctx.save_for_backward(mem, fast_mem, wd)
        ctx.maps, ctx.params = maps, (W, b)
        return frames

    @staticmethod
    def backward(ctx, g):
        _arm()
        mem, fast_mem, wd = ctx.saved_tensors
        maps = ctx.maps
        g = g.contiguous()
        d, dt, dev = g.shape[1], g.dtype, g.device
        n_vis = maps.F * maps.hw
        g_vis = torch.empty((n_vis, d), dtype=dt, device=dev)
        ops.rows_copy(g, maps.vis_dst, g_vis, None, n_vis)
        d_fast = ops.linear_fwd(g_vis, wd) if ctx.needs_input_grad[1] else None
        mix = torch.empty((n_vis, d), dtype=dt, device=dev)
        ops.rows_copy(mem, maps.vis_src, mix, None, n_vis, add=fast_mem)
        dW, db = _wgrad(g_vis, mix, _can_defer(*ctx.params), want_bias=True)
        d_mem = None
        if ctx.needs_input_grad[0]:
            d_mem = torch.empty_like(mem)
            ops.rows_segment_sum(g, maps.seg_txt[0], maps.seg_txt[1], d_mem, maps.clip_txt)
            G = torch.empty((maps.n * maps.hw, d), dtype=dt, device=dev)
            ops.rows_segment_sum(g, maps.seg_vis[0], maps.seg_vis[1], G)
            ops.linear_ex(G, wd, None, residual=G, res_map=maps.iota_vis, out=d_mem, out_map=maps.clip_vis)
        return d_mem, d_fast, dW, db, None


class AttnCoreFn(Function):

    @staticmethod
    def forward(ctx, q, k, v, key_pad, B, Lq, Lk, H, p_drop, seed):
        E = q.shape[1]
        scale = 1.0 / math.sqrt(E // H)
        q3, k3, v3 = q.view(B, Lq, E), k.view(B, Lk, E), v.view(B, Lk, E)
        out, probs, _ = ops.mha_fwd(q3, k3, v3, key_pad, H, scale, need_wavg=False, dropout_p=p_drop, seed=seed)
        ctx.save_for_backward(q3, k3, v3, probs)
        ctx.cfg = (B, Lq, Lk, H, E, scale, p_drop, seed)
        return out.view(B * Lq, E)

    @staticmethod
    def backward(ctx, dout):
        q3, k3, v3, probs = ctx.saved_tensors
        B, Lq, Lk, H, E, scale, p_drop, seed = ctx.cfg
        dq, dk, dv = torch.empty_like(q3), torch.empty_like(k3), torch.empty_like(v3)
        ops.mha_bwd(q3, k3, v3, dout.contiguous().view(B, Lq, E), probs, None, H, scale, dq, dk, dv, dropout_p=p_drop, seed=seed)
        return dq.view(B * Lq, E), dk.view(B * Lk, E), dv.view(B * Lk, E), None, None, None, None, None, None, None


def attention_core(q, k, v, key_pad, B, Lq, Lk, H, dropout_p=0.0, training=False):
    p = dropout_p if training else 0.0
    return AttnCoreFn.apply(q, k, v, key_pad, B, Lq, Lk, H, p, _seed() if p > 0 else 0)


def multihead_attention(q_in, k_in, v_in, W_in, b_in, W_out, b_out, key_pad, B, Lq, Lk, H, need_weights=False,
                        attn_dropout=0.0, out_dropout=0.0, training=False, q_pos=None):
    pa = attn_dropout if training else 0.0
    po = out_dropout if training else 0.0
    return MHAFn.apply(q_in, q_pos, k_in, v_in, W_in, b_in, W_out, b_out, key_pad, B, Lq, Lk, H, need_weights,
                       pa, _seed() if pa > 0 else 0, po, _seed() if po > 0 else 0)


class GeluFn(Function):

    @staticmethod
    def forward(ctx, x):
        x = x.contiguous()
        ctx.save_for_backward(x)
        return ops.gelu_fwd(x)

    @staticmethod
    def backward(ctx, g):
        (x,) = ctx.saved_tensors
        return ops.gelu_bwd(g.contiguous(), x)


def gelu(x):
    return GeluFn.apply(x)


class DropoutFn(Function):
    @staticmethod
    def forward(ctx, x, p, seed):
        ctx.cfg = (p, seed)
        return ops.dropout(x.contiguous(), p, seed)

    @staticmethod
    def backward(ctx, g):
        p, seed = ctx.cfg
        return ops.dropout(g.contiguous(), p, seed), None, None


def dropout(x, p, training):
    if not training or p <= 0:
        return x
    return DropoutFn.apply(x, p, _seed())


class CastFn(Function):

    @staticmethod
    def forward(ctx, x, dtype):
        ctx.src = x.dtype
        return ops.cast(x.contiguous(), dtype)

    @staticmethod
    def backward(ctx, g):
        return ops.cast(g.contiguous(), ctx.src), None


def cast(x, dtype):
    return x if x.dtype == dtype else CastFn.apply(x, dtype)
```

### tubedetr_amd/models/transformer.py

```python
from __future__ import annotations

import copy
import math
import os
from typing import List, Optional

import torch
from torch import Tensor, nn

from .. import functional as Fk
from .. import ops as _ops
from ..util.misc import LRUCache
from .position_encoding import TimeEmbeddingLearned, TimeEmbeddingSine

FAST_MODES_IN_HIP = ("",)
FAST_MODES = ("", "gating", "transformer", "pool", "noslow")


class MultiheadAttention(nn.Module):

    def __init__(self, embed_dim: int, num_heads: int, dropout: float = 0.0):
        super().__init__()
        self.embed_dim, self.num_heads, self.dropout = embed_dim, num_heads, dropout
        self.in_proj_weight = nn.Parameter(torch.empty(3 * embed_dim, embed_dim))
        self.in_proj_bias = nn.Parameter(torch.zeros(3 * embed_dim))
        self.out_proj = nn.Linear(embed_dim, embed_dim)
        nn.init.xavier_uniform_(self.in_proj_weight)
        nn.init.constant_(self.out_proj.bias, 0.0)

    def run_prekv(self, q_in, kv, layer, key_pad, B, Lq, Lk, need_weights, out_dropout, training, q_pos=None):
        return Fk.multihead_attention_prekv(q_in, kv, layer, self.in_proj_weight, self.in_proj_bias, self.out_proj.weight, self.out_proj.bias, key_pad,
                                            B, Lq, Lk, self.num_heads, need_weights, attn_dropout=self.dropout, out_dropout=out_dropout, training=training,
                                            q_pos=q_pos)

    def run_q1(self, q_in, anchor, key_pad, F, S, need_weights, out_dropout, training, q_pos=None):
        return Fk.multihead_attention_q1(q_in, anchor, self.in_proj_weight, self.in_proj_bias, self.out_proj.weight, self.out_proj.bias, key_pad,
                                         F, S, self.num_heads, need_weights, attn_dropout=self.dropout, out_dropout=out_dropout, training=training,
                                         q_pos=q_pos)

    def run(self, q_in, k_in, v_in, key_pad, B, Lq, Lk, need_weights, out_dropout, training, q_pos=None):
        return Fk.multihead_attention(q_in, k_in, v_in, self.in_proj_weight, self.in_proj_bias, self.out_proj.weight,
                                      self.out_proj.bias, key_pad, B, Lq, Lk, self.num_heads, need_weights,
                                      attn_dropout=self.dropout, out_dropout=out_dropout, training=training, q_pos=q_pos)


class TransformerEncoderLayer(nn.Module):
    def __init__(self, d_model, nhead, dim_feedforward=2048, dropout=0.1, activation="relu"):
        super().__init__()
        if activation != "relu":
            raise NotImplementedError("only the reference default activation (relu) is fused in the HIP FFN")
        self.self_attn = MultiheadAttention(d_model, nhead, dropout=dropout)
        self.linear1 = nn.Linear(d_model, dim_feedforward)
        self.linear2 = nn.Linear(dim_feedforward, d_model)
        self.norm1 = nn.LayerNorm(d_model)
        self.norm2 = nn.LayerNorm(d_model)
        self.p = dropout

    def forward(self, src: Tensor, pos: Optional[Tensor], key_pad: Optional[Tensor], B: int, S: int) -> Tensor:
        a, _ = self.self_attn.run(src, None, src, key_pad, B, S, S, False, self.p, self.training, q_pos=pos)
        src = Fk.add_layernorm(a, src, self.norm1.weight, self.norm1.bias, self.norm1.eps)
        f = Fk.ffn(src, self.linear1.weight, self.linear1.bias, self.linear2.weight, self.linear2.bias, self.p, self.training)
        return Fk.add_layernorm(f, src, self.norm2.weight, self.norm2.bias, self.norm2.eps)


class TransformerEncoder(nn.Module):
    def __init__(self, encoder_layer, num_layers, norm=None, return_weights=False):
        super().__init__()
        self.layers = nn.ModuleList([copy.deepcopy(encoder_layer) for _ in range(num_layers)])
        self.num_layers = num_layers
        self.norm = norm
        self.return_weights = return_weights

    def forward(self, src, key_pad, pos, B, S):
        out = src
        for layer in self.layers:
            out = layer(out, pos, key_pad, B, S)
        if self.norm is not None:
            out = Fk.add_layernorm(out, None, self.norm.weight, self.norm.bias, self.norm.eps)
        return out


class TransformerDecoderLayer(nn.Module):
    def __init__(self, d_model, nhead, dim_feedforward=2048, dropout=0.1, activation="relu", no_tsa=False):
        super().__init__()
        if activation != "relu":
            raise NotImplementedError("only relu")
        self.self_attn = MultiheadAttention(d_model, nhead, dropout=dropout)
        self.cross_attn_image = MultiheadAttention(d_model, nhead, dropout=dropout)
        self.linear1 = nn.Linear(d_model, dim_feedforward)
        self.linear2 = nn.Linear(dim_feedforward, d_model)
        self.norm1 = nn.LayerNorm(d_model)
        self.norm3 = nn.LayerNorm(d_model)
        self.norm4 = nn.LayerNorm(d_model)
        self.p = dropout
        self.no_tsa = no_tsa

    def forward(self, tgt, query_pos, mem, pos, query_mask, memory_mask, b: int, t: int, S: int, kv=None, index: int = 0):
        if self.no_tsa:
            a, w = self.self_attn.run(tgt, None, tgt, None, b * t, 1, 1, True, self.p, self.training, q_pos=query_pos)
        else:
            a, w = self.self_attn.run(tgt, None, tgt, query_mask, b, t, t, True, self.p, self.training, q_pos=query_pos)
        tgt = Fk.add_layernorm(a, tgt, self.norm1.weight, self.norm1.bias, self.norm1.eps)
        if isinstance(kv, tuple) and len(kv) == 2:
            a, cw = self.cross_attn_image.run_q1(tgt, kv, memory_mask, b * t, S, True, self.p, self.training, q_pos=query_pos)
        elif kv is not None:
            a, cw = self.cross_attn_image.run_prekv(tgt, kv, index, memory_mask, b * t, 1, S, True, self.p, self.training, q_pos=query_pos)
        else:
            mem_k = Fk.AddFn.apply(mem, pos) if pos is not None else mem
            a, cw = self.cross_attn_image.run(tgt, mem_k, mem, memory_mask, b * t, 1, S, True, self.p, self.training, q_pos=query_pos)
        tgt = Fk.add_layernorm(a, tgt, self.norm3.weight, self.norm3.bias, self.norm3.eps)
        f = Fk.ffn(tgt, self.linear1.weight, self.linear1.bias, self.linear2.weight, self.linear2.bias, self.p, self.training)
        tgt = Fk.add_layernorm(f, tgt, self.norm4.weight, self.norm4.bias, self.norm4.eps)
        return tgt, w, cw


class TransformerDecoder(nn.Module):
    def __init__(self, decoder_layer, num_layers, norm=None, return_intermediate=False, return_weights=False):
        super().__init__()
        self.layers = nn.ModuleList([copy.deepcopy(decoder_layer) for _ in range(num_layers)])
        self.num_layers = num_layers
        self.norm = norm
        self.return_intermediate = return_intermediate
        self.return_weights = return_weights

    def forward(self, tgt, query_pos, mem, pos, query_mask, memory_mask, b, t, S):
        inter, ws, cws = [], [], []
        out = tgt
        att = self.layers[0].cross_attn_image
        if (os.environ.get("TD_CROSS_Q1", "1") != "0" and att.embed_dim == 256 and att.num_heads == 8 and S <= 320
                and not (pos is not None and pos.requires_grad)):
            kv = Fk.cross_q1_memory(mem, pos)
        else:
            kv = Fk.cross_kv(mem, pos, [l.cross_attn_image for l in self.layers]) if os.environ.get("TD_KV_HOIST", "1") != "0" else None
        for i, layer in enumerate(self.layers):
            out, w, cw = layer(out, query_pos, mem, pos, query_mask, memory_mask, b, t, S, kv=kv, index=i)
            if self.return_intermediate:
                inter.append(Fk.add_layernorm(out, None, self.norm.weight, self.norm.bias, self.norm.eps))
                ws.append(w)
                cws.append(cw)
        if not self.return_intermediate:
            out = Fk.add_layernorm(out, None, self.norm.weight, self.norm.bias, self.norm.eps) if self.norm is not None else out
            return (out, w, cw) if self.return_weights else out
        hs = torch.stack(inter)
        if not self.return_weights:
            return hs
        return hs, torch.stack(ws), torch.stack(cws)


class FeatureResizer(nn.Module):

    def __init__(self, input_feat_size, output_feat_size, dropout, do_ln=True):
        super().__init__()
        self.do_ln = do_ln
        self.fc = nn.Linear(input_feat_size, output_feat_size, bias=True)
        self.layer_norm = nn.LayerNorm(output_feat_size, eps=1e-12)
        self.p = dropout

    def forward(self, rows: Tensor) -> Tensor:
        x = Fk.linear(rows, self.fc.weight, self.fc.bias)
        if self.do_ln:
            x = Fk.add_layernorm(x, None, self.layer_norm.weight, self.layer_norm.bias, self.layer_norm.eps)
        return Fk.dropout(x, self.p, self.training)


class HashTokenizer:

    def batch_encode_plus(self, text: List[str], padding="longest", return_tensors="pt"):
        import zlib

        from transformers import BatchEncoding

        rows = [[0] + [3 + zlib.crc32(w.encode()) % 49990 for w in s.split()] + [2] for s in text]
        L = max(len(r) for r in rows)
        ids = torch.tensor([r + [1] * (L - len(r)) for r in rows], dtype=torch.long)
        att = torch.tensor([[1] * len(r) + [0] * (L - len(r)) for r in rows], dtype=torch.long)
        be = BatchEncoding({"input_ids": ids, "attention_mask": att})
        be._encodings = [None] * len(text)
        return be


def _load_text_encoder(name: str):
    import os
    import warnings

    from transformers import RobertaConfig, RobertaModel, RobertaTokenizerFast

    try:
        tok = RobertaTokenizerFast.from_pretrained(name, local_files_only=True)
        enc = RobertaModel.from_pretrained(name, local_files_only=True)
        return tok, enc
    except Exception as exc:
        if os.environ.get("TD_ALLOW_RANDOM_TEXT_ENCODER", "0") != "1":
            raise RuntimeError(
                f"text encoder {name!r} could not be loaded ({type(exc).__name__}: {exc}); the reference needs the pretrained "
                "files too.  For synthetic benchmarks / tests without them set TD_ALLOW_RANDOM_TEXT_ENCODER=1 (random-init "
# ... 292 lines not shown
```

### tubedetr_amd/ops.py

```python
from __future__ import annotations

import os

import ctypes as C
from typing import Optional, Tuple

import torch

from . import _hip
from ._hip import ConvDesc, Epilogue, check, dtype_code, ptr, stream_ptr

Tensor = torch.Tensor


class _ZeroArena:

    def __init__(self, chunk: int):
        self.chunk = chunk
        self.buf = None
        self.off = 0

    def take(self, shape, device) -> torch.Tensor:
        n = 1
        for d_ in shape:
# ... 131 lines not shown
        while len(self.slots) < self.RING:
            self.slots.append([torch.empty(self.cap, dtype=torch.uint8, pin_memory=True),
                               torch.empty(self.cap, dtype=torch.uint8, device=device), None])

    def take(self, nbytes: int, device):
        capturing = torch.cuda.is_current_stream_capturing()
        if capturing:
            ok = [s for s in self.slots if s[0].numel() >= nbytes and s[1].device == device]
            if not ok:
                raise RuntimeError("td job tables must exist before a stream capture: run one training step eagerly first")
            slot = ok[0]
            self.slots.remove(slot)
            self.retired.append(slot)
            return slot[0], slot[1], (lambda: None)
        if len(self.slots) < self.RING or self.cap < nbytes:
            self._grow(nbytes, device)
        slot = self.slots[self.next % len(self.slots)]
        self.next += 1
        if slot[2] is not None:
            slot[2].synchronize()

        def done():
            ev = torch.cuda.Event()
            ev.record()
            slot[2] = ev

        return slot[0], slot[1], done


job_tables = _JobTables()


def conv_wgrad_batch(jobs) -> list:
    jobs = list(jobs)
    arr = (_hip.WgradJob * len(jobs))()
    outs = []
    for a, (g, x, R, S, stride, pad, scale, ci_real) in zip(arr, jobs):
        N, H, W, Cs = x.shape
        _, Ho, Wo, Co = g.shape
        assert g.is_contiguous() and x.is_contiguous() and g.dtype == x.dtype
        dw = torch.empty((Co, ci_real, R, S), dtype=torch.float32, device=x.device)
        outs.append(dw)
        a.g, a.src, a.dW, a.scale = g.data_ptr(), x.data_ptr(), dw.data_ptr(), (scale.data_ptr() if scale is not None else None)
        a.d = _desc(N, H, W, Cs, Ho, Wo, R, S, stride, pad, 0, Co, Co)
        a.ldg, a.ci_real, a.dbias = Co, ci_real, None
    nbytes = _hip.lib().td_conv_wgrad_batch_table_bytes(len(jobs))
    th, td_, done = job_tables.take(nbytes, jobs[0][0].device)
    check(_hip.lib().td_conv_wgrad_batch(arr, len(jobs), dtype_code(jobs[0][0].dtype), th.data_ptr(), td_.data_ptr(), nbytes, stream_ptr()),
          "td_conv_wgrad_batch")
    done()
    return outs


def linear_wgrad_batch(jobs) -> None:
    if not jobs:
        return
    key0 = (jobs[0][0].dtype, jobs[0][0].device)
    if any((j[0].dtype, j[0].device) != key0 for j in jobs):
        groups: dict = {}
        for j in jobs:
            groups.setdefault((j[0].dtype, j[0].device), []).append(j)
        for sub in groups.values():
            linear_wgrad_batch(sub)
        return
    arr = (_hip.WgradJob * len(jobs))()
    for a, job in zip(arr, jobs):
        g, x, dw_ptr, db_ptr = job[:4]
        M, K = x.shape
        Nn = g.shape[1]
        assert g.shape[0] == M and g.stride(1) == 1 and x.is_contiguous() and g.dtype == x.dtype
        a.g, a.src, a.dW, a.scale, a.dbias = g.data_ptr(), x.data_ptr(), dw_ptr, None, db_ptr
        a.d = _desc(1, M, 1, K, M, 1, 1, 1, 1, 0, 0, Nn, Nn)
        a.ldg, a.ci_real = g.stride(0), K
        a.accumulate = int(len(job) > 4 and bool(job[4]))
    nbytes = _hip.lib().td_conv_wgrad_batch_table_bytes(len(jobs))
    dev = jobs[0][0].device
    th, td_, done = job_tables.take(nbytes, dev)
    check(_hip.lib().td_conv_wgrad_batch(arr, len(jobs), dtype_code(jobs[0][0].dtype), th.data_ptr(), td_.data_ptr(), nbytes, stream_ptr()),
          "td_conv_wgrad_batch(linears)")
    done()


def linear_fwd(x: Tensor, w: Tensor, bias: Optional[Tensor] = None, *, residual=None, relu=False, sigmoid=False,
               mask_src=None, dropout_p=0.0, seed=0, alpha=1.0, out: Optional[Tensor] = None) -> Tensor:
    M, K = x.shape
    Nn = w.shape[0]
    assert w.shape[1] == K and w.dtype == x.dtype and x.is_contiguous() and w.is_contiguous()
    y = out if out is not None else torch.empty((M, Nn), dtype=x.dtype, device=x.device)
    conv_gemm_raw(x, w, y, _desc(1, M, 1, K, M, 1, 1, 1, 1, 0, 0, Nn, Nn), _epi(bias, residual, mask_src, relu, sigmoid, dropout_p, seed, alpha))
    return y


def pw_chain2(y2: Tensor, w3: Tensor, b3: Tensor, residual: Tensor, w1: Tensor, b1: Tensor, *, out: Optional[Tensor] = None,
              h1: Optional[Tensor] = None) -> Tuple[Tensor, Tensor]:
    M, P = y2.shape
    assert y2.dtype == torch.bfloat16 and w3.shape == (4 * P, P) and w1.shape == (P, 4 * P) and residual.shape == (M, 4 * P)
    assert y2.is_contiguous() and w3.is_contiguous() and w1.is_contiguous() and residual.is_contiguous()
    assert b3.dtype == torch.float32 and b1.dtype == torch.float32 and b3.numel() == 4 * P and b1.numel() == P
    out = out if out is not None else torch.empty((M, 4 * P), dtype=y2.dtype, device=y2.device)
    h1 = h1 if h1 is not None else torch.empty((M, P), dtype=y2.dtype, device=y2.device)
    check(_hip.lib().td_pw_chain2(ptr(y2), ptr(w3), ptr(b3), ptr(residual), ptr(out), ptr(w1), ptr(b1), ptr(h1), M, P, dtype_code(y2.dtype),
                                  stream_ptr()), "td_pw_chain2")
    return out, h1


def _rows2d(t: Tensor):
    assert t.dim() == 2 and t.stride(1) == 1, "row-major 2-D operand expected (unit column stride)"
    return t


def linear_ex(a1: Tensor, w: Tensor, bias: Optional[Tensor] = None, *, a2: Optional[Tensor] = None, a1_map: Optional[Tensor] = None,
              a2_map: Optional[Tensor] = None, w_shared: bool = False, out: Optional[Tensor] = None, out_map: Optional[Tensor] = None,
              out_rows: Optional[int] = None, residual: Optional[Tensor] = None, res_map: Optional[Tensor] = None, relu=False, mask_src=None,
              dropout_p=0.0, seed=0, alpha=1.0) -> Tensor:
    _rows2d(a1)
    K1 = a1.shape[1]
    K2 = _rows2d(a2).shape[1] if a2 is not None else 0
    M = int(a1_map.numel()) if a1_map is not None else a1.shape[0]
    Nn = w.shape[0]
    assert w.is_contiguous() and w.dtype == a1.dtype and w.shape[1] == (K1 if (w_shared or a2 is None) else K1 + K2)
    for m_ in (a1_map, a2_map, out_map, res_map):
        assert m_ is None or (m_.dtype == torch.int32 and m_.is_contiguous() and m_.numel() == M)
    if out is None:
        out = torch.empty((out_rows if out_rows is not None else M, Nn), dtype=a1.dtype, device=a1.device)
    _rows2d(out)
    x = _hip.LinearExDesc()
    x.M, x.N, x.K1, x.K2 = M, Nn, K1, K2
    x.lda1, x.lda2, x.ldc = a1.stride(0), (a2.stride(0) if a2 is not None else 0), out.stride(0)
    x.ldr = _rows2d(residual).stride(0) if residual is not None else 0
    x.w_shared = int(bool(w_shared and a2 is not None))
    x.rows1, x.rows2 = a1.shape[0], (a2.shape[0] if a2 is not None else 0)
    x.a1_map, x.a2_map, x.out_map, x.res_map = ptr(a1_map), ptr(a2_map), ptr(out_map), ptr(res_map)
    epi = _epi(bias, residual, mask_src, relu, False, dropout_p, seed, alpha)
    check(_hip.lib().td_linear_ex(ptr(a1), ptr(a2), ptr(w), ptr(out), C.byref(x), C.byref(epi), dtype_code(a1.dtype), stream_ptr()), "td_linear_ex")
    return out


def rows_copy(src: Tensor, src_map: Optional[Tensor], dst: Tensor, dst_map: Optional[Tensor], n_rows: int, add: Optional[Tensor] = None) -> Tensor:
    _rows2d(src), _rows2d(dst)
    cols = src.shape[1]
    assert dst.shape[1] == cols and dst.dtype == src.dtype and (add is None or (_rows2d(add).shape[1] == cols and add.dtype == src.dtype and add.shape[0] >= n_rows))
    for m_ in (src_map, dst_map):
        assert m_ is None or (m_.dtype == torch.int32 and m_.is_contiguous() and m_.numel() == n_rows)
    check(_hip.lib().td_rows_copy(ptr(src), ptr(src_map), ptr(add), ptr(dst), ptr(dst_map), n_rows, cols, src.stride(0), add.stride(0) if add is not None else 0,
                                  dst.stride(0), dtype_code(src.dtype), stream_ptr()), "td_rows_copy")
    return dst


def rows_segment_sum(inp: Tensor, idx: Tensor, seg_ptr: Tensor, out: Tensor, out_map: Optional[Tensor] = None) -> Tensor:
    _rows2d(inp), _rows2d(out)
    n_out = seg_ptr.numel() - 1
    assert idx.dtype == torch.int32 and seg_ptr.dtype == torch.int32 and out.dtype == inp.dtype and out.shape[1] == inp.shape[1]
    assert out_map is None or (out_map.dtype == torch.int32 and out_map.numel() == n_out)
    check(_hip.lib().td_rows_segment_sum(ptr(inp), ptr(idx), ptr(seg_ptr), ptr(out), ptr(out_map), n_out, inp.shape[1], inp.stride(0), out.stride(0),
                                         dtype_code(inp.dtype), stream_ptr()), "td_rows_segment_sum")
    return out


def linear_wgrad(g: Tensor, x: Tensor, *, out: Optional[Tensor] = None, splits: int = 0, dbias: Optional[Tensor] = None) -> Tensor:
    M, K = x.shape
    Nn = g.shape[1]
    dw = out if out is not None else zeros_f32((Nn, K), x.device)
    d = _desc(1, M, 1, K, M, 1, 1, 1, 1, 0, 0, Nn, Nn)
    if dbias is not None:
        assert dbias.dtype == torch.float32 and dbias.numel() == Nn and dbias.is_contiguous()
    assert g.stride(1) == 1 and x.is_contiguous()
    check(_hip.lib().td_conv_wgrad_bias(ptr(g), ptr(x), ptr(dw), ptr(dbias), C.byref(d), g.stride(0), dtype_code(x.dtype), splits, stream_ptr()),
          "td_conv_wgrad")
    return dw


def weight_prep(W: Tensor, dtype: torch.dtype, *, bn=None, bias: Optional[Tensor] = None, need_dgrad: bool = True, cpad: Optional[int] = None):
# ... 261 lines not shown
```

Baseline: 106.3.

## Fold residual-gradient accumulation into the backward input-projection GEMM epilogues

Adds a post-add epilogue mode to the pointwise GEMM kernels: the mask operand slot carries a previous tensor that is added to the rounded output. The transformer encoder and decoder layers use it to add the residual-branch gradient directly inside the dx GEMMs of FFN and attention backward. The add-layernorm backward then stops returning a separate residual gradient, so autograd no longer runs separate accumulation adds. This saves elementwise kernels and memory traffic, but adds new kernel instantiations and an extra bf16 rounding before the add.

```diff
diff --git a/include/tubedetr_hip.h b/include/tubedetr_hip.h
--- a/include/tubedetr_hip.h
+++ b/include/tubedetr_hip.h
@@ -67,6 +67,8 @@
 
 int td_conv_gemm(const void* src, const void* wmat, void* out, const td_conv_desc* d, const td_epilogue* e,
                  int dtype, td_stream_t stream);
+int td_conv_gemm_acc(const void* src, const void* wmat, void* out, const td_conv_desc* d, const td_epilogue* e, const void* prev,
+                     int dtype, td_stream_t stream);
 
 typedef struct td_linear_ex_desc {
   int M, N, K1, K2;
diff --git a/tubedetr_amd/_hip.py b/tubedetr_amd/_hip.py
--- a/tubedetr_amd/_hip.py
+++ b/tubedetr_amd/_hip.py
@@ -68,6 +68,7 @@
     "td_prof_collect": [_I, _I, C.POINTER(C.c_longlong), C.POINTER(C.c_double), C.POINTER(C.c_double)],
     "td_prof_collect_bytes": [_I, _I, C.POINTER(C.c_double)],
     "td_conv_gemm": [_P, _P, _P, C.POINTER(ConvDesc), C.POINTER(Epilogue), _I, _P],
+    "td_conv_gemm_acc": [_P, _P, _P, C.POINTER(ConvDesc), C.POINTER(Epilogue), _P, _I, _P],
     "td_conv_wgrad": [_P, _P, _P, C.POINTER(ConvDesc), _I, _I, _I, _P],
     "td_conv_wgrad_bias": [_P, _P, _P, _P, C.POINTER(ConvDesc), _I, _I, _I, _P],
     "td_conv_wgrad_batch": [C.POINTER(WgradJob), _I, _I, _P, _P, _SZ, _P],
diff --git a/tubedetr_amd/csrc/gemm_conv.hip b/tubedetr_amd/csrc/gemm_conv.hip
--- a/tubedetr_amd/csrc/gemm_conv.hip
+++ b/tubedetr_amd/csrc/gemm_conv.hip
@@ -43,6 +43,7 @@
   int w_ld;
   int wtap[4];
   int use_wtap;
+  int post_add;
 };
 
 template <typename T>
@@ -114,6 +115,13 @@
 template <>
 __device__ __forceinline__ uint4 pack16<u16>(const float (&v)[8]) {
   return make_uint4(pack_bf16x2(v[0], v[1]), pack_bf16x2(v[2], v[3]), pack_bf16x2(v[4], v[5]), pack_bf16x2(v[6], v[7]));
+}
+template <typename T>
+__device__ __forceinline__ void post_add16(float (&v)[16 / sizeof(T)], const float (&prev)[16 / sizeof(T)]) {
+  float q[16 / sizeof(T)];
+  unpack16<T>(pack16<T>(v), q);
+#pragma unroll
+  for (int i = 0; i < (int)(16 / sizeof(T)); ++i) v[i] = q[i] + prev[i];
 }
 template <typename T>
 __device__ __forceinline__ void store4(char* base, size_t off, const float (&v)[4]);
@@ -154,7 +162,7 @@
 #endif
 }
 
-template <typename T, int BM, int BN, int NST, bool PW, bool TU = false, bool GX = false>
+template <typename T, int BM, int BN, int NST, bool PW, bool TU = false, bool GX = false, bool PA = false>
 __global__ __launch_bounds__(256, (BM * BN >= 128 * 128 || NST == 3) ? 2 : 3) void conv_gemm_kernel(GemmParams p) {
   static_assert(!(PW && TU), "pointwise layers have no taps");
   static_assert(!GX || (PW && NST == 2), "the gather-extended operand is a pointwise, two-stage instance");
@@ -484,8 +492,13 @@
       if (p.mask_src) {
         float m8[EPL];
         unpack16<T>(msk[it], m8);
-#pragma unroll
-        for (int r = 0; r < EPL; ++r) v[r] = m8[r] > 0.f ? v[r] : 0.f;
+        constexpr bool PADD = PW && !TU && !GX && (ES == 2 || PA);
+        if (PADD && p.post_add) {
+          post_add16<T>(v, m8);
+        } else {
+#pragma unroll
+          for (int r = 0; r < EPL; ++r) v[r] = m8[r] > 0.f ? v[r] : 0.f;
+        }
       }
       if (p.drop_thresh) {
 #pragma unroll
@@ -837,17 +850,18 @@
         asm volatile("ds_read_b128 %0, %1 offset:1024" : "=v"(o1) : "v"(sra) : "memory");
       }
       if (p.mask_src) {
+        const bool padd = !TU && p.post_add != 0;
         float x8[8], m8[8];
         unpack16<T>(make_uint4(s0.x, s0.y, s0.z, s0.w), x8);
         unpack16<T>(mk[b][0], m8);
 #pragma unroll
-        for (int r = 0; r < 8; ++r) x8[r] = m8[r] > 0.f ? x8[r] : 0.f;
+        for (int r = 0; r < 8; ++r) x8[r] = padd ? x8[r] + m8[r] : (m8[r] > 0.f ? x8[r] : 0.f);
         const uint4 q0 = pack16<T>(x8);
         s0 = u32x4_t{q0.x, q0.y, q0.z, q0.w};
         unpack16<T>(make_uint4(s1.x, s1.y, s1.z, s1.w), x8);
         unpack16<T>(mk[b][1], m8);
 #pragma unroll
-        for (int r = 0; r < 8; ++r) x8[r] = m8[r] > 0.f ? x8[r] : 0.f;
+        for (int r = 0; r < 8; ++r) x8[r] = padd ? x8[r] + m8[r] : (m8[r] > 0.f ? x8[r] : 0.f);
         const uint4 q1 = pack16<T>(x8);
         s1 = u32x4_t{q1.x, q1.y, q1.z, q1.w};
       }
@@ -1111,8 +1125,12 @@
       if (p.mask_src) {
         float m8[EPL];
         unpack16<T>(msk[b][it], m8);
-#pragma unroll
-        for (int r = 0; r < EPL; ++r) v[r] = m8[r] > 0.f ? v[r] : 0.f;
+        if (p.post_add) {
+          post_add16<T>(v, m8);
+        } else {
+#pragma unroll
+          for (int r = 0; r < EPL; ++r) v[r] = m8[r] > 0.f ? v[r] : 0.f;
+        }
       }
       if (live[b][it]) st16(p.out + offs[b][it] * ES, pack16<T>(v));
     }
@@ -1122,8 +1140,9 @@
 #undef TD_STAMP
 }
 
-template <int NKT, bool RES, bool MSK>
+template <int NKT, bool RES, bool MSK, bool PA = false>
 __global__ __launch_bounds__(256, 2) void pw_resident2_kernel(GemmParams p, int MT, int P) {
+  static_assert(!PA || (MSK && !RES), "post-add instances: prev in the mask slot, no residual");
   using T = u16;
   constexpr int ES = 2;
   constexpr uint32_t OOB = 0xFFFFFFF0u;
@@ -1278,8 +1297,12 @@
         if constexpr (MSK) {
           float m8[EPL];
           unpack16<T>(make_uint4(msk[RB][it].x, msk[RB][it].y, msk[RB][it].z, msk[RB][it].w), m8);
-#pragma unroll
-          for (int r = 0; r < EPL; ++r) v[r] = m8[r] > 0.f ? v[r] : 0.f;
+          if constexpr (PA) {
+            post_add16<T>(v, m8);
+          } else {
+#pragma unroll
+            for (int r = 0; r < EPL; ++r) v[r] = m8[r] > 0.f ? v[r] : 0.f;
+          }
         }
         if (p.drop_thresh) {
 #pragma unroll
@@ -2094,7 +2117,7 @@
   size_t w_bytes;
 };
 static int conv_gemm_launch(const void* src, const void* wmat, void* out, const td_conv_desc* d, const td_epilogue* e, int dtype,
-                            td_stream_t stream, const WeightSubset* sub);
+                            td_stream_t stream, const WeightSubset* sub, const void* prev = nullptr);
 
 static int conv_dgrad_s2_by_parity(const void* g, const void* w_dgrad, void* dx, const td_conv_desc* d, const td_epilogue* e, int dtype,
                                    td_stream_t stream) {
@@ -2142,8 +2165,18 @@
   return conv_gemm_launch(src, wmat, out, d, e, dtype, stream, nullptr);
 }
 
+extern "C" int td_conv_gemm_acc(const void* src, const void* wmat, void* out, const td_conv_desc* d, const td_epilogue* e, const void* prev,
+                                int dtype, td_stream_t stream) {
+  TD_REQUIRE(src && wmat && out && d && prev, "td_conv_gemm_acc: null pointer");
+  TD_REQUIRE(d->R == 1 && d->S == 1 && d->stride == 1 && d->pad == 0 && d->out_sp <= 1 && !d->aniso && d->Hs == d->Ho && d->Ws == d->Wo,
+             "td_conv_gemm_acc: pointwise layers with dense output rows only");
+  TD_REQUIRE(!(e && (e->mask_src || e->residual || e->dropout_p > 0.f)), "td_conv_gemm_acc: no mask operand (its slot carries prev), no residual, no dropout");
+  TD_REQUIRE(d->Nc % (dtype == TD_BF16 ? 8 : 4) == 0 && d->ldc % (dtype == TD_BF16 ? 8 : 4) == 0, "td_conv_gemm_acc: Nc and ldc must be multiples of 16 bytes");
+  return conv_gemm_launch(src, wmat, out, d, e, dtype, stream, nullptr, prev);
+}
+
 static int conv_gemm_launch(const void* src, const void* wmat, void* out, const td_conv_desc* d, const td_epilogue* e, int dtype,
-                            td_stream_t stream, const WeightSubset* sub) {
+                            td_stream_t stream, const WeightSubset* sub, const void* prev) {
   TD_REQUIRE(src && wmat && out && d, "td_conv_gemm: null pointer");
   int rc = validate(d, dtype, "td_conv_gemm");
   if (rc) return rc;
@@ -2188,6 +2221,10 @@
     }
   }
   TD_REQUIRE(d->ldc >= d->Nc, "td_conv_gemm: ldc < Nc");
+  if (prev) {
+    p.mask_src = (const char*)prev;
+    p.post_add = 1;
+  }
   hipStream_t st = (hipStream_t)stream;
   static const int n_cu = [] {
     int dev = 0, cus = 256;
@@ -2221,7 +2258,8 @@
       dim3 g2(2 * n_cu);
 #define TD_PWR(NK)                                                                               \
   do {                                                                                           \
-    if (hr && hm) pw_resident2_kernel<NK, true, true><<<g2, 256, 0, st>>>(p, MTp, Pp);          \
+    if (p.post_add) pw_resident2_kernel<NK, false, true, true><<<g2, 256, 0, st>>>(p, MTp, Pp); \
+    else if (hr && hm) pw_resident2_kernel<NK, true, true><<<g2, 256, 0, st>>>(p, MTp, Pp);     \
     else if (hr) pw_resident2_kernel<NK, true, false><<<g2, 256, 0, st>>>(p, MTp, Pp);          \
     else if (hm) pw_resident2_kernel<NK, false, true><<<g2, 256, 0, st>>>(p, MTp, Pp);          \
     else pw_resident2_kernel<NK, false, false><<<g2, 256, 0, st>>>(p, MTp, Pp);                 \
@@ -2305,6 +2343,10 @@
     else if (deep_ok) conv_gemm_kernel<u16, 64, 128, 3, false><<<grid, 256, 0, st>>>(p);
     else if (small_m) TD_LAUNCH(u16, 64, 128);
     else TD_LAUNCH(u16, 128, 128);
+  } else if (p.post_add) {
+    if (narrow) conv_gemm_kernel<float, 128, 64, 2, true, false, false, true><<<grid, 256, 0, st>>>(p);
+    else if (small_m) conv_gemm_kernel<float, 64, 128, 2, true, false, false, true><<<grid, 256, 0, st>>>(p);
+    else conv_gemm_kernel<float, 128, 128, 2, true, false, false, true><<<grid, 256, 0, st>>>(p);
   } else {
     if (narrow) TD_LAUNCH(float, 128, 64);
     else if (small_m) TD_LAUNCH(float, 64, 128);
diff --git a/tubedetr_amd/functional.py b/tubedetr_amd/functional.py
--- a/tubedetr_amd/functional.py
+++ b/tubedetr_amd/functional.py
@@ -235,6 +235,17 @@
     return dW, db
 
 
+_FOLD_RES = [_os.environ.get("TD_FOLD_RESIDUAL", "1") != "0"]
+
+
+def set_residual_fold(on: bool) -> None:
+    _FOLD_RES[0] = bool(on)
+
+
+def residual_fold_on(*pos) -> bool:
+    return _FOLD_RES[0] and not any(q is not None and q.requires_grad for q in pos)
+
+
 class LinearFn(Function):
 
     @staticmethod
@@ -289,8 +300,9 @@
 class FFNFn(Function):
 
     @staticmethod
-    def forward(ctx, x, W1, b1, W2, b2, p: float, seed1: int, seed2: int):
+    def forward(ctx, x, W1, b1, W2, b2, p: float, seed1: int, seed2: int, fold: bool = False):
         _note_use(ctx.needs_input_grad[1], W1, b1, W2, b2)
+        ctx.fold = fold
         w1f, w1d, _, _ = prepared(W1, x.dtype)
         w2f, w2d, _, _ = prepared(W2, x.dtype)
         h = ops.linear_fwd(x, w1f, b1.detach(), relu=True, dropout_p=p, seed=seed1)
@@ -306,37 +318,38 @@
         x, h, w1d, w2d = ctx.saved_tensors
         p, seed1, seed2 = ctx.cfg
         defer = _can_defer(*ctx.params)
-        g2 = ops.dropout(dy.contiguous(), p, seed2) if p > 0 else dy.contiguous()
+        dy = dy.contiguous()
+        g2 = ops.dropout(dy, p, seed2) if p > 0 else dy
         dW2, db2 = _wgrad(g2, h, defer, want_bias=True)
         dh = ops.linear_fwd(g2, w2d, mask_src=h, alpha=1.0 / (1.0 - p) if p > 0 else 1.0)
         dW1, db1 = _wgrad(dh, x, defer, want_bias=True)
-        dx = ops.linear_fwd(dh, w1d) if ctx.needs_input_grad[0] else None
-        return dx, dW1, db1, dW2, db2, None, None, None
-
-
-def ffn(x, W1, b1, W2, b2, dropout_p=0.0, training=False):
+        dx = ops.linear_fwd(dh, w1d, acc_prev=dy if ctx.fold else None) if ctx.needs_input_grad[0] else None
+        return dx, dW1, db1, dW2, db2, None, None, None, None
+
+
+def ffn(x, W1, b1, W2, b2, dropout_p=0.0, training=False, fold_residual=False):
     p = dropout_p if training else 0.0
-    return FFNFn.apply(x, W1, b1, W2, b2, p, _seed() if p > 0 else 0, _seed() if p > 0 else 0)
+    return FFNFn.apply(x, W1, b1, W2, b2, p, _seed() if p > 0 else 0, _seed() if p > 0 else 0, bool(fold_residual))
 
 
 class AddLayerNormFn(Function):
 
     @staticmethod
-    def forward(ctx, x, r, gamma, beta, eps: float):
+    def forward(ctx, x, r, gamma, beta, eps: float, r_folded: bool = False):
         y, s, mean, rstd = ops.add_layernorm_fwd(x, r, gamma.detach(), beta.detach(), eps)
         ctx.save_for_backward(s, mean, rstd, gamma.detach())
-        ctx.has_r = r is not None
+        ctx.has_r = r is not None and not r_folded
         return y
 
     @staticmethod
     def backward(ctx, dy):
         s, mean, rstd, gamma = ctx.saved_tensors
         ds, dg, db = ops.add_layernorm_bwd(dy.contiguous(), s, mean, rstd, gamma)
-        return ds, (ds if ctx.has_r else None), dg, db, None
-
-
-def add_layernorm(x, r, gamma, beta, eps=1e-5):
-    return AddLayerNormFn.apply(x, r, gamma, beta, eps)
+        return ds, (ds if ctx.has_r else None), dg, db, None, None
+
+
+def add_layernorm(x, r, gamma, beta, eps=1e-5, r_grad_folded=False):
+    return AddLayerNormFn.apply(x, r, gamma, beta, eps, bool(r_grad_folded))
 
 
 class AddFn(Function):
@@ -353,8 +366,10 @@
 class MHAFn(Function):
 
     @staticmethod
-    def forward(ctx, q_in, q_pos, k_in, v_in, W_in, b_in, W_out, b_out, key_pad, B, Lq, Lk, H, need_w, p_attn, seed_attn, p_out, seed_out):
+    def forward(ctx, q_in, q_pos, k_in, v_in, W_in, b_in, W_out, b_out, key_pad, B, Lq, Lk, H, need_w, p_attn, seed_attn, p_out, seed_out, fold: int = 0):
         _note_use(ctx.needs_input_grad[4], W_in, b_in, W_out, b_out)
+        assert not (fold and q_pos is not None and ctx.needs_input_grad[1]), "a positional operand with a gradient cannot share the folded sum"
+        ctx.fold = fold
         E = q_in.shape[1]
         dt = q_in.dtype
         same_qk = k_in is None
@@ -400,7 +415,8 @@
         dt = q_in.dtype
         dev = q_in.device
         defer = _can_defer(*ctx.params)
-        g = ops.dropout(dout.contiguous(), p_out, seed_out) if p_out > 0 else dout.contiguous()
+        dout = dout.contiguous()
+        g = ops.dropout(dout, p_out, seed_out) if p_out > 0 else dout
         if defer:
             dW_in = torch.empty((3 * E, E), dtype=torch.float32, device=dev)
             db_in = torch.empty(3 * E, dtype=torch.float32, device=dev)
@@ -423,24 +439,28 @@
             ops.mha_bwd(q, k, v, dctx, probs, dwa, H, scale, dq, dk, dv, dropout_p=p_attn, seed=seed_attn)
         dv2 = dv.view(B * Lk, E)
         _wgrad(dv2, v_in, defer, want_bias=True, out=dW_in[2 * E :], dbias=db_in[2 * E :])
-        d_v_in = ops.linear_fwd(dv2, wv_d) if ctx.needs_input_grad[3] else None
+        fold_v = ctx.fold == 2 and ctx.needs_input_grad[0]
+        d_v_in = ops.linear_fwd(dv2, wv_d) if (ctx.needs_input_grad[3] and not fold_v) else None
         d_q_in = d_k_in = None
         need_q = ctx.needs_input_grad[0] or (q_pos is not None and ctx.needs_input_grad[1])
+        acc = dout if ctx.fold else None
         if same_qk:
             dqk2 = dqk.view(B * Lq, 2 * E)
             _wgrad(dqk2, q_in, defer, want_bias=True, out=dW_in[: 2 * E], dbias=db_in[: 2 * E], x2=q_pos)
             if need_q:
-                d_q_in = ops.linear_fwd(dqk2, wd_list[0])
+                d_q_in = ops.linear_fwd(dqk2, wd_list[0], acc_prev=acc)
         else:
             dq2, dk2 = dq.view(B * Lq, E), dk.view(B * Lk, E)
             _wgrad(dq2, q_in, defer, want_bias=True, out=dW_in[:E], dbias=db_in[:E], x2=q_pos)
             _wgrad(dk2, k_in, defer, want_bias=True, out=dW_in[E : 2 * E], dbias=db_in[E : 2 * E])
             if need_q:
-                d_q_in = ops.linear_fwd(dq2, wd_list[0])
+                d_q_in = ops.linear_fwd(dq2, wd_list[0], acc_prev=acc)
             if ctx.needs_input_grad[2]:
                 d_k_in = ops.linear_fwd(dk2, wd_list[1])
+        if fold_v:
+            d_q_in = ops.linear_fwd(dv2, wv_d, acc_prev=d_q_in)
         return (d_q_in if ctx.needs_input_grad[0] else None, d_q_in if (q_pos is not None and ctx.needs_input_grad[1]) else None, d_k_in, d_v_in,
-                dW_in, db_in, dW_out, db_out) + (None,) * 10
+                dW_in, db_in, dW_out, db_out) + (None,) * 11
 
 
 class _CrossKVShared:
@@ -504,8 +524,11 @@
 class MHAPreKVFn(Function):
 
     @staticmethod
-    def forward(ctx, q_in, q_pos, K_all, V_all, W_in, b_in, W_out, b_out, key_pad, shared, layer, B, Lq, Lk, H, need_w, p_attn, seed_attn, p_out, seed_out):
+    def forward(ctx, q_in, q_pos, K_all, V_all, W_in, b_in, W_out, b_out, key_pad, shared, layer, B, Lq, Lk, H, need_w, p_attn, seed_attn, p_out, seed_out,
+                fold: bool = False):
         _note_use(ctx.needs_input_grad[4], W_in, b_in, W_out, b_out)
+        assert not (fold and q_pos is not None and ctx.needs_input_grad[1]), "a positional operand with a gradient cannot share the folded sum"
+        ctx.fold = fold
         E = q_in.shape[1]
         dt = q_in.dtype
         nl = shared.n_layers
@@ -535,7 +558,8 @@
         nl = sh.n_layers
         dt, dev = q_in.dtype, q_in.device
         defer = _can_defer(*ctx.params)
-        g = ops.dropout(dout.contiguous(), p_out, seed_out) if p_out > 0 else dout.contiguous()
+        dout = dout.contiguous()
+        g = ops.dropout(dout, p_out, seed_out) if p_out > 0 else dout
         if defer:
             dW_in = torch.empty((3 * E, E), dtype=torch.float32, device=dev)
             db_in = torch.empty(3 * E, dtype=torch.float32, device=dev)
@@ -559,8 +583,8 @@
         _wgrad(dK_all[:, cols], sh.mem, defer, want_bias=True, out=dW_in[E : 2 * E], dbias=db_in[E : 2 * E], x2=sh.pos)
         _wgrad(dV_all[:, cols], sh.mem, defer, want_bias=True, out=dW_in[2 * E :], dbias=db_in[2 * E :])
         need_pos = q_pos is not None and ctx.needs_input_grad[1]
-        d_q_in = ops.linear_fwd(dq2, wq_d) if (ctx.needs_input_grad[0] or need_pos) else None
-        return (d_q_in if ctx.needs_input_grad[0] else None, d_q_in if need_pos else None, None, None, dW_in, db_in, dW_out, db_out) + (None,) * 12
+        d_q_in = ops.linear_fwd(dq2, wq_d, acc_prev=dout if ctx.fold else None) if (ctx.needs_input_grad[0] or need_pos) else None
+        return (d_q_in if ctx.needs_input_grad[0] else None, d_q_in if need_pos else None, None, None, dW_in, db_in, dW_out, db_out) + (None,) * 13
 
 
 class _CrossQ1Shared:
@@ -606,8 +630,10 @@
 class CrossQ1Fn(Function):
 
     @staticmethod
-    def forward(ctx, q_in, q_pos, token, W_in, b_in, W_out, b_out, key_pad, shared, F, S, H, need_w, p_attn, seed_attn, p_out, seed_out):
+    def forward(ctx, q_in, q_pos, token, W_in, b_in, W_out, b_out, key_pad, shared, F, S, H, need_w, p_attn, seed_attn, p_out, seed_out, fold: bool = False):
         _note_use(ctx.needs_input_grad[3], W_in, b_in, W_out, b_out)
+        assert not (fold and q_pos is not None and ctx.needs_input_grad[1]), "a positional operand with a gradient cannot share the folded sum"
+        ctx.fold = fold
         E = q_in.shape[1]
         dt = q_in.dtype
         scale = 1.0 / math.sqrt(E // H)
@@ -638,7 +664,8 @@
         sh = ctx.shared
         dt, dev = q_in.dtype, q_in.device
         defer = _can_defer(*ctx.params)
-        g = ops.dropout(dout.contiguous(), p_out, seed_out) if p_out > 0 else dout.contiguous()
+        dout = dout.contiguous()
+        g = ops.dropout(dout, p_out, seed_out) if p_out > 0 else dout
         dW_in = torch.empty((3 * E, E), dtype=torch.float32, device=dev)
         db_in = torch.empty(3 * E, dtype=torch.float32, device=dev)
         dW_out, db_out = _wgrad(g, ctxv, defer, want_bias=True)
@@ -675,8 +702,8 @@
             db_in[:E].zero_()
             _wgrad(dq, q_in, False, want_bias=True, out=dW_in[:E], dbias=db_in[:E], x2=q_pos)
         need_pos = q_pos is not None and ctx.needs_input_grad[1]
-        d_q_in = ops.linear_fwd(dq, wq_d) if (ctx.needs_input_grad[0] or need_pos) else None
-        return (d_q_in if ctx.needs_input_grad[0] else None, d_q_in if need_pos else None, None, dW_in, db_in, dW_out, db_out) + (None,) * 10
+        d_q_in = ops.linear_fwd(dq, wq_d, acc_prev=dout if ctx.fold else None) if (ctx.needs_input_grad[0] or need_pos) else None
+        return (d_q_in if ctx.needs_input_grad[0] else None, d_q_in if need_pos else None, None, dW_in, db_in, dW_out, db_out) + (None,) * 11
 
 
 _CROSS_DMEM_DEFER = _os.environ.get("TD_CROSS_DMEM_DEFER", "1") != "0"
@@ -688,12 +715,12 @@
 
 
 def multihead_attention_q1(q_in, anchor, W_in, b_in, W_out, b_out, key_pad, F, S, H, need_weights=True, attn_dropout=0.0, out_dropout=0.0,
-                           training=False, q_pos=None):
+                           training=False, q_pos=None, fold_residual=False):
     pa = attn_dropout if training else 0.0
     po = out_dropout if training else 0.0
     token, shared = anchor
     return CrossQ1Fn.apply(q_in, q_pos, token, W_in, b_in, W_out, b_out, key_pad, shared, F, S, H, need_weights,
-                           pa, _seed() if pa > 0 else 0, po, _seed() if po > 0 else 0)
+                           pa, _seed() if pa > 0 else 0, po, _seed() if po > 0 else 0, bool(fold_residual))
 
 
 def cross_kv(mem, pos, attn_modules):
@@ -707,12 +734,12 @@
 
 
 def multihead_attention_prekv(q_in, kv, layer, W_in, b_in, W_out, b_out, key_pad, B, Lq, Lk, H, need_weights=False, attn_dropout=0.0,
-                              out_dropout=0.0, training=False, q_pos=None):
+                              out_dropout=0.0, training=False, q_pos=None, fold_residual=False):
     pa = attn_dropout if training else 0.0
     po = out_dropout if training else 0.0
     K_all, V_all, shared = kv
     return MHAPreKVFn.apply(q_in, q_pos, K_all, V_all, W_in, b_in, W_out, b_out, key_pad, shared, layer, B, Lq, Lk, H, need_weights,
-                            pa, _seed() if pa > 0 else 0, po, _seed() if po > 0 else 0)
+                            pa, _seed() if pa > 0 else 0, po, _seed() if po > 0 else 0, bool(fold_residual))
 
 
 class ReplicaMaps:
@@ -837,11 +864,12 @@
 
 
 def multihead_attention(q_in, k_in, v_in, W_in, b_in, W_out, b_out, key_pad, B, Lq, Lk, H, need_weights=False,
-                        attn_dropout=0.0, out_dropout=0.0, training=False, q_pos=None):
+                        attn_dropout=0.0, out_dropout=0.0, training=False, q_pos=None, fold_residual=False):
     pa = attn_dropout if training else 0.0
     po = out_dropout if training else 0.0
+    fold = 0 if not fold_residual else (2 if v_in is q_in else 1)
     return MHAFn.apply(q_in, q_pos, k_in, v_in, W_in, b_in, W_out, b_out, key_pad, B, Lq, Lk, H, need_weights,
-                       pa, _seed() if pa > 0 else 0, po, _seed() if po > 0 else 0)
+                       pa, _seed() if pa > 0 else 0, po, _seed() if po > 0 else 0, fold)
 
 
 class GeluFn(Function):
diff --git a/tubedetr_amd/models/transformer.py b/tubedetr_amd/models/transformer.py
--- a/tubedetr_amd/models/transformer.py
+++ b/tubedetr_amd/models/transformer.py
@@ -28,20 +28,20 @@
         nn.init.xavier_uniform_(self.in_proj_weight)
         nn.init.constant_(self.out_proj.bias, 0.0)
 
-    def run_prekv(self, q_in, kv, layer, key_pad, B, Lq, Lk, need_weights, out_dropout, training, q_pos=None):
+    def run_prekv(self, q_in, kv, layer, key_pad, B, Lq, Lk, need_weights, out_dropout, training, q_pos=None, fold_residual=False):
         return Fk.multihead_attention_prekv(q_in, kv, layer, self.in_proj_weight, self.in_proj_bias, self.out_proj.weight, self.out_proj.bias, key_pad,
                                             B, Lq, Lk, self.num_heads, need_weights, attn_dropout=self.dropout, out_dropout=out_dropout, training=training,
-                                            q_pos=q_pos)
-
-    def run_q1(self, q_in, anchor, key_pad, F, S, need_weights, out_dropout, training, q_pos=None):
+                                            q_pos=q_pos, fold_residual=fold_residual)
+
+    def run_q1(self, q_in, anchor, key_pad, F, S, need_weights, out_dropout, training, q_pos=None, fold_residual=False):
         return Fk.multihead_attention_q1(q_in, anchor, self.in_proj_weight, self.in_proj_bias, self.out_proj.weight, self.out_proj.bias, key_pad,
                                          F, S, self.num_heads, need_weights, attn_dropout=self.dropout, out_dropout=out_dropout, training=training,
-                                         q_pos=q_pos)
-
-    def run(self, q_in, k_in, v_in, key_pad, B, Lq, Lk, need_weights, out_dropout, training, q_pos=None):
+                                         q_pos=q_pos, fold_residual=fold_residual)
+
+    def run(self, q_in, k_in, v_in, key_pad, B, Lq, Lk, need_weights, out_dropout, training, q_pos=None, fold_residual=False):
         return Fk.multihead_attention(q_in, k_in, v_in, self.in_proj_weight, self.in_proj_bias, self.out_proj.weight,
                                       self.out_proj.bias, key_pad, B, Lq, Lk, self.num_heads, need_weights,
-                                      attn_dropout=self.dropout, out_dropout=out_dropout, training=training, q_pos=q_pos)
+                                      attn_dropout=self.dropout, out_dropout=out_dropout, training=training, q_pos=q_pos, fold_residual=fold_residual)
 
 
 class TransformerEncoderLayer(nn.Module):
@@ -57,10 +57,11 @@
         self.p = dropout
 
     def forward(self, src: Tensor, pos: Optional[Tensor], key_pad: Optional[Tensor], B: int, S: int) -> Tensor:
-        a, _ = self.self_attn.run(src, None, src, key_pad, B, S, S, False, self.p, self.training, q_pos=pos)
-        src = Fk.add_layernorm(a, src, self.norm1.weight, self.norm1.bias, self.norm1.eps)
-        f = Fk.ffn(src, self.linear1.weight, self.linear1.bias, self.linear2.weight, self.linear2.bias, self.p, self.training)
-        return Fk.add_layernorm(f, src, self.norm2.weight, self.norm2.bias, self.norm2.eps)
+        fold = Fk.residual_fold_on(pos)
+        a, _ = self.self_attn.run(src, None, src, key_pad, B, S, S, False, self.p, self.training, q_pos=pos, fold_residual=fold)
+        src = Fk.add_layernorm(a, src, self.norm1.weight, self.norm1.bias, self.norm1.eps, r_grad_folded=fold)
+        f = Fk.ffn(src, self.linear1.weight, self.linear1.bias, self.linear2.weight, self.linear2.bias, self.p, self.training, fold_residual=fold)
+        return Fk.add_layernorm(f, src, self.norm2.weight, self.norm2.bias, self.norm2.eps, r_grad_folded=fold)
 
 
 class TransformerEncoder(nn.Module):
@@ -96,21 +97,22 @@
         self.no_tsa = no_tsa
 
     def forward(self, tgt, query_pos, mem, pos, query_mask, memory_mask, b: int, t: int, S: int, kv=None, index: int = 0):
+        fold, fold_ffn = Fk.residual_fold_on(query_pos), Fk.residual_fold_on()
         if self.no_tsa:
-            a, w = self.self_attn.run(tgt, None, tgt, None, b * t, 1, 1, True, self.p, self.training, q_pos=query_pos)
-        else:
-            a, w = self.self_attn.run(tgt, None, tgt, query_mask, b, t, t, True, self.p, self.training, q_pos=query_pos)
-        tgt = Fk.add_layernorm(a, tgt, self.norm1.weight, self.norm1.bias, self.norm1.eps)
+            a, w = self.self_attn.run(tgt, None, tgt, None, b * t, 1, 1, True, self.p, self.training, q_pos=query_pos, fold_residual=fold)
+        else:
+            a, w = self.self_attn.run(tgt, None, tgt, query_mask, b, t, t, True, self.p, self.training, q_pos=query_pos, fold_residual=fold)
+        tgt = Fk.add_layernorm(a, tgt, self.norm1.weight, self.norm1.bias, self.norm1.eps, r_grad_folded=fold)
         if isinstance(kv, tuple) and len(kv) == 2:
-            a, cw = self.cross_attn_image.run_q1(tgt, kv, memory_mask, b * t, S, True, self.p, self.training, q_pos=query_pos)
+            a, cw = self.cross_attn_image.run_q1(tgt, kv, memory_mask, b * t, S, True, self.p, self.training, q_pos=query_pos, fold_residual=fold)
         elif kv is not None:
-            a, cw = self.cross_attn_image.run_prekv(tgt, kv, index, memory_mask, b * t, 1, S, True, self.p, self.training, q_pos=query_pos)
+            a, cw = self.cross_attn_image.run_prekv(tgt, kv, index, memory_mask, b * t, 1, S, True, self.p, self.training, q_pos=query_pos, fold_residual=fold)
         else:
             mem_k = Fk.AddFn.apply(mem, pos) if pos is not None else mem
-            a, cw = self.cross_attn_image.run(tgt, mem_k, mem, memory_mask, b * t, 1, S, True, self.p, self.training, q_pos=query_pos)
-        tgt = Fk.add_layernorm(a, tgt, self.norm3.weight, self.norm3.bias, self.norm3.eps)
-        f = Fk.ffn(tgt, self.linear1.weight, self.linear1.bias, self.linear2.weight, self.linear2.bias, self.p, self.training)
-        tgt = Fk.add_layernorm(f, tgt, self.norm4.weight, self.norm4.bias, self.norm4.eps)
+            a, cw = self.cross_attn_image.run(tgt, mem_k, mem, memory_mask, b * t, 1, S, True, self.p, self.training, q_pos=query_pos, fold_residual=fold)
+        tgt = Fk.add_layernorm(a, tgt, self.norm3.weight, self.norm3.bias, self.norm3.eps, r_grad_folded=fold)
+        f = Fk.ffn(tgt, self.linear1.weight, self.linear1.bias, self.linear2.weight, self.linear2.bias, self.p, self.training, fold_residual=fold_ffn)
+        tgt = Fk.add_layernorm(f, tgt, self.norm4.weight, self.norm4.bias, self.norm4.eps, r_grad_folded=fold_ffn)
         return tgt, w, cw
 
 
diff --git a/tubedetr_amd/ops.py b/tubedetr_amd/ops.py
--- a/tubedetr_amd/ops.py
+++ b/tubedetr_amd/ops.py
@@ -237,12 +237,18 @@
 
 
 def linear_fwd(x: Tensor, w: Tensor, bias: Optional[Tensor] = None, *, residual=None, relu=False, sigmoid=False,
-               mask_src=None, dropout_p=0.0, seed=0, alpha=1.0, out: Optional[Tensor] = None) -> Tensor:
+               mask_src=None, dropout_p=0.0, seed=0, alpha=1.0, out: Optional[Tensor] = None, acc_prev: Optional[Tensor] = None) -> Tensor:
     M, K = x.shape
     Nn = w.shape[0]
     assert w.shape[1] == K and w.dtype == x.dtype and x.is_contiguous() and w.is_contiguous()
     y = out if out is not None else torch.empty((M, Nn), dtype=x.dtype, device=x.device)
-    conv_gemm_raw(x, w, y, _desc(1, M, 1, K, M, 1, 1, 1, 1, 0, 0, Nn, Nn), _epi(bias, residual, mask_src, relu, sigmoid, dropout_p, seed, alpha))
+    desc, epi = _desc(1, M, 1, K, M, 1, 1, 1, 1, 0, 0, Nn, Nn), _epi(bias, residual, mask_src, relu, sigmoid, dropout_p, seed, alpha)
+    if acc_prev is None:
+        conv_gemm_raw(x, w, y, desc, epi)
+    else:
+        assert mask_src is None and acc_prev.shape == (M, Nn) and acc_prev.dtype == x.dtype and acc_prev.is_contiguous()
+        check(_hip.lib().td_conv_gemm_acc(ptr(x), ptr(w), ptr(y), C.byref(desc), C.byref(epi), ptr(acc_prev), dtype_code(x.dtype), stream_ptr()),
+              "td_conv_gemm_acc")
     return y
 
 
```

After: 106.3. No clear change (-0.0%).
